# rikuu/Gap2Seq

Measured on AMD Instinct MI355X. Metric: gaps filled/sec (whole node), k=31 synthetic 3 Mbp DBG, higher is better.
Workload: dtype u32

## Files before the change

### gap2seq_amd/csrc/d3_device.h

```cpp
#pragma once
#include <hip/hip_runtime_api.h>
#include <stdint.h>

#include "d2_device.h"
#include "fill_device.h"

#define G2S_D3_BLOCK_VARS 16u
#define G2S_RAND_BLOCK 4096u
#define G2S_RAND_WINDOW 160u
#define G2S_D3_TABLE_BUDGET (8u << 20)

#define G2S_D3_UNHANDLED 0x1u
#define G2S_D3_BUDGET 0x2u
#define G2S_D3_ANOMALY 0x4u

namespace g2s {

struct D3Gap {
  uint64_t arena_off;
  int32_t skip_thr;
  uint16_t lmf;
  uint8_t kind;
  uint8_t pad;
};

struct D3HostItem {
  uint32_t gap, n_segs;
  uint64_t seg_off;
  uint64_t rnd_off;
  uint32_t draws;
  uint32_t pad;
};
struct D3Side {
  D3HostItem* items = nullptr;
  GapOut* outs = nullptr;
  SegRec* segs = nullptr;
  uint32_t* rnd = nullptr;
  uint64_t cap_items = 0, cap_segs = 0, cap_rnd = 0;
  unsigned long long* count = nullptr;
};

struct alignas(16) D3Var {
  uint32_t gap, R, toff, tile0;
  uint32_t base, dmin, dspread, ns;
  uint64_t sub_at;
  uint32_t start_seg, start_t;
  int32_t len0, len1, n_len;
  uint32_t pad;
};
struct alignas(16) D3Trace {
  uint64_t arena_off;
  uint64_t sub_at;
  uint32_t gi;
  uint32_t off, want;
  uint16_t lmf, nsegs;
};
static_assert(sizeof(D3Var) == 64 && sizeof(D3Trace) == 32, "record layouts");

struct D3Summary {
  uint32_t status, unhandled, n_var, anomalies;
  unsigned long long host_items, host_segs, host_rnd;
  uint32_t handoff_waves, tiles;
  uint64_t table_entries, block_entries;
  uint64_t draws_min, draws_spread, draws_total;
  uint64_t xA, sA, xB, sB, xD, sD, segs, fill_bytes;
  uint32_t seg_gaps, filled;
  uint32_t rand_state[31];
  uint32_t trace_waves;
  uint32_t big_gaps;
  uint32_t traced_gaps;
  uint32_t spec_gaps;
  uint32_t handoff_gaps;
};
static_assert(sizeof(D3Summary) <= 512, "the lap stamps live at byte 512 of the summary's slot");

struct RandTables {
  const uint32_t* hi = nullptr;
  const uint32_t* mid = nullptr;
  const uint32_t* lane = nullptr;
};
void rand_tables_host(uint32_t* hi , uint32_t* mid , uint32_t* lane );

struct D3Work {
  uint32_t* ginfo = nullptr;
  uint32_t* dmin = nullptr;
  uint32_t* dspread = nullptr;
  uint32_t* base = nullptr;
  uint32_t* vrank = nullptr;
  uint32_t* var_gap = nullptr;
  uint32_t* var_R = nullptr;
  uint32_t* var_toff = nullptr;
  uint32_t* var_tile = nullptr;
  uint32_t* blk_toff = nullptr;
  uint32_t* blk_in = nullptr;
  uint32_t* dvar = nullptr;
  int32_t* skip = nullptr;
  uint32_t* tile_var = nullptr;
  D3Var* vdesc = nullptr;
  D3Trace* tdesc = nullptr;
  uint32_t* host_slot = nullptr;
  D3HostItem* hitems = nullptr;
  uint16_t* tab = nullptr;
  uint32_t* btab = nullptr;
  D3Summary* sum = nullptr;
  unsigned long long* fill_bytes = nullptr;
  uint32_t* link = nullptr;
  const D2Out* d2out = nullptr;
  const uint32_t* d2runs = nullptr;
  uint64_t* hops = nullptr;
  const char* spec_text = nullptr;
  const uint32_t* spec_res = nullptr;
  uint8_t* tab_bad = nullptr;
};
size_t d3_work_bytes(uint32_t n);
void d3_work_carve(void* p, uint32_t n, D3Work* w);

struct D3Params {
  int32_t k, skip_confident, all_paths, unique_paths;
  uint64_t max_states;
  uint64_t arena_base;
  uint32_t n;
  uint32_t has_skip;
  uint32_t seg_cap;
  uint32_t map_cap;
  uint32_t group_size;
  uint64_t sub_region;
  uint32_t laps;
  uint32_t self_clean;
  uint32_t base0, R0, d_in;
  const unsigned long long* d2_done;
  uint32_t d2_wgs;
  uint32_t restart;
};

hipError_t launch_rand_fill(hipStream_t st, uint32_t* rnd_all, const RandTables& rt, const D3Summary* sum_dev, uint64_t capacity,
                            uint64_t first_value = 0);

hipError_t launch_d3_sharded_classes(hipStream_t st, const D3Params& P, const D3Work& W, const GapOut* outs, const D3Gap* dgaps,
                                     bool summary_is_clean);
hipError_t launch_d3_sharded_tables(hipStream_t st, const D3Params& P, const D3Work& W, const GapOut* outs, const SubRec* sub,
                                    uint32_t* rnd_all, uint64_t rnd_capacity, uint32_t* group_fn );
hipError_t launch_d3_sharded_trace(hipStream_t st, const D3Params& P, const D3Work& W, const GapOut* outs, const SubRec* sub,
                                   const char* lastch_up, const char* lastch_dn, uint32_t* rnd_all, uint64_t rnd_capacity,
                                   void* results, char* arena, const D3Side& side, void* summary_host,
                                   hipEvent_t ev_d2 = nullptr );

hipError_t launch_rand_window(hipStream_t st, uint32_t* rnd_all, const uint32_t* link);

hipError_t launch_d3(hipStream_t st, const D3Params& P, const D3Work& W, const GapDev* gaps, const GapOut* outs,
                     const D3Gap* dgaps, const SubRec* sub, const char* lastch_up, const char* lastch_dn,
                     const RandTables& rt, uint32_t* rnd_all ,
                     uint64_t rnd_capacity, void* results ,
                     char* arena , const D3Side& side ,
                     void* summary_host ,
                     bool summary_is_clean ,
                     uint32_t* clean_words ,
                     hipEvent_t ev_chain = nullptr ,
                     hipEvent_t ev_d2 = nullptr ,
                     hipEvent_t ev_stop = nullptr );

hipError_t test_d3_tables(const uint32_t* segs, uint32_t nsegs, int32_t n_len, int32_t len0, int32_t len1, uint32_t start_seg,
                          const uint32_t* rnd, uint64_t rnd_cap, uint32_t base, uint32_t R, uint32_t dmin, uint32_t dspread,
                          uint16_t* entries, uint8_t* bad, uint32_t* anomalies);

uint64_t d3_chain_launches();

}
```

### gap2seq_amd/csrc/d3_device.hip

```cpp
#include "sync_debug.h"
#include <hip/hip_runtime.h>
#include <hip/hip_ext.h>

#include <algorithm>
#include <atomic>
#include <cstddef>
#include <cstdlib>
#include <cstring>
#include <mutex>
#include <set>
#include <vector>

#include "../../include/g2s.h"
#include "d3_device.h"
#include "envcache.hpp"

namespace {

using g2s::D3Gap;
using g2s::D3Params;
using g2s::D3Summary;
using g2s::D3Work;

__device__ __forceinline__ uint32_t uni(uint32_t x) { return (uint32_t)__builtin_amdgcn_readfirstlane((int)x); }

#define GI_CLASS(x) ((x) & 3u)
#define GI_FILLED 0x4u
#define GI_SKIPPED 0x8u
#define GI_BAD 0x10u
#define GI_MEM 0x20u
#define GI_PHASE_D 0x40u
#define D3_TILE 256u
#define GI_HOST 0x80u

__device__ __forceinline__ void stamp(const D3Work& W, int slot) {
  ((unsigned long long*)((char*)W.sum + 512))[slot] = wall_clock64();
}

__device__ __forceinline__ const SubRec* sub_of(const D3Params& P, const SubRec* sub, uint32_t i) {
  return sub + (uint64_t)(i / P.group_size) * P.sub_region;
}

__device__ __forceinline__ int gap_count(const GapOut& go, const D3Params& P, bool phase_d) {
  if (phase_d && !P.skip_confident && P.all_paths) return go.count_s;
  return go.c_count;
}

__device__ __forceinline__ uint32_t dpp_scan_add(uint32_t x) {
  x += (uint32_t)__builtin_amdgcn_update_dpp(0, (int)x, 0x111, 0xF, 0xF, false);
  x += (uint32_t)__builtin_amdgcn_update_dpp(0, (int)x, 0x112, 0xF, 0xF, false);
  x += (uint32_t)__builtin_amdgcn_update_dpp(0, (int)x, 0x114, 0xF, 0xF, false);
  x += (uint32_t)__builtin_amdgcn_update_dpp(0, (int)x, 0x118, 0xF, 0xF, false);
  x += (uint32_t)__builtin_amdgcn_update_dpp(0, (int)x, 0x142, 0xA, 0xF, false);
  x += (uint32_t)__builtin_amdgcn_update_dpp(0, (int)x, 0x143, 0xC, 0xF, false);
  return x;
}
__device__ __forceinline__ uint32_t sat_add(uint32_t a, uint32_t b) { const uint32_t t = a + b; return t < a ? 0xFFFFFFFFu : t; }
__device__ __forceinline__ uint32_t dpp_scan_sat(uint32_t x) {
  x = sat_add(x, (uint32_t)__builtin_amdgcn_update_dpp(0, (int)x, 0x111, 0xF, 0xF, false));
  x = sat_add(x, (uint32_t)__builtin_amdgcn_update_dpp(0, (int)x, 0x112, 0xF, 0xF, false));
  x = sat_add(x, (uint32_t)__builtin_amdgcn_update_dpp(0, (int)x, 0x114, 0xF, 0xF, false));
  x = sat_add(x, (uint32_t)__builtin_amdgcn_update_dpp(0, (int)x, 0x118, 0xF, 0xF, false));
  x = sat_add(x, (uint32_t)__builtin_amdgcn_update_dpp(0, (int)x, 0x142, 0xA, 0xF, false));
  x = sat_add(x, (uint32_t)__builtin_amdgcn_update_dpp(0, (int)x, 0x143, 0xC, 0xF, false));
  return x;
}
__device__ __forceinline__ uint32_t dpp_sum(uint32_t x) { return (uint32_t)__builtin_amdgcn_readlane((int)dpp_scan_add(x), 63); }
__device__ __forceinline__ unsigned long long wave_add64(unsigned long long v) {
  const unsigned long long lo = dpp_sum((uint32_t)v & 0xFFFFFFu), mid = dpp_sum((uint32_t)(v >> 24) & 0xFFFFFFu), hi = dpp_sum((uint32_t)(v >> 48));
  return lo + (mid << 24) + (hi << 48);
}

__device__ __forceinline__ uint32_t d3_classify_body(const D3Params& P, const D3Work& W, const GapOut* __restrict__ outs,
                                                     const D3Gap* __restrict__ dgaps, uint32_t first, uint32_t stride,
                                                     uint32_t* l_gi, uint32_t* l_dm, uint32_t* l_ds, int32_t* l_sk,
                                                     unsigned long long* red, bool one_wg) {
  const uint32_t n = P.n;
  unsigned long long xA = 0, sA = 0, xB = 0, sB = 0, xD = 0, sD = 0, segs = 0;
  uint32_t unhandled = 0, seg_gaps = 0, big = 0, traced = 0, spec = 0, handoff = 0;
  for (uint32_t i = first; i < n; i += stride) {
    const D3Gap dg = dgaps[i];
    const GapOut& go = outs[i];
    const uint32_t flags = go.flags, n_states = go.n_states, n_right = go.n_right, x_right = go.x_right, x_left = go.x_left;
    const uint32_t x_sub = go.x_sub, n_sub = go.n_sub, nseg_b = go.stat[3], dflags = go.dflags, stop0 = go.stop[0], stop1 = go.stop[1];
    const int c_count = go.c_count, n_len = go.n_len, len0 = go.len[0], len1 = go.len[1], reached_j = go.reached_j, count_s = go.count_s;
    const uint32_t n_xl = go.n_xl;
    const uint64_t sub_off = go.sub_off;
    uint32_t gi = 0, dmin = 0, spread = 0;
    if (dg.kind != 0) gi = GI_BAD;
    else {
      if (flags & (G2S_DEV_OVERFLOW_A | G2S_DEV_OVERFLOW_B)) unhandled++;
      else if ((uint64_t)n_states > P.max_states || (uint64_t)n_right > P.max_states) gi = GI_MEM;
      else {
        xA += x_right; sA += n_right; xB += x_left; sB += n_states; xD += x_sub; sD += n_sub;
        segs += nseg_b;
        seg_gaps++;
        if (flags & G2S_DEV_BIG) big++;
        if (dflags & G2S_DEVA_TRACED) traced++;
        if (dflags & G2S_DEVA_SPEC) spec++;
        const bool phase_d = c_count > 0 && n_len > 0;
        const bool by_host = phase_d && !(dflags & (G2S_DEVA_ANALYSED | G2S_DEVA_D2_PENDING));
        const int cnt = (phase_d && !P.skip_confident && P.all_paths) ? count_s : c_count;
        if (cnt > 0 && (!P.unique_paths || cnt == 1)) gi |= GI_FILLED;
        if (n_len > 0) gi |= ((uint32_t)reached_j & 0xFFu) << 8;
        if (phase_d) {
          gi |= GI_PHASE_D;
          if (by_host) gi |= GI_HOST;
          if (by_host || (!P.skip_confident && (dflags & G2S_DEVA_D2_PENDING))) handoff++;
          int lo_d = 0x7FFFFFFF, hi_d = 0;
#pragma unroll
          for (int q = 0; q < 2; q++) {
            if (q >= n_len) continue;
            const uint32_t sw = q ? stop1 : stop0;
            const int lq = q ? len1 : len0;
            int lo = (int)(sw & 0xFFFFu), hi = (int)(sw >> 16);
            if (lo > hi || hi > (int)dg.lmf) { lo = 0; hi = (int)dg.lmf; }
            lo_d = min(lo_d, 1 + lq - hi);
            hi_d = max(hi_d, 1 + lq - lo);
          }
          lo_d = max(lo_d, 1);
          hi_d = max(hi_d, lo_d);
          dmin = (uint32_t)lo_d;
          spread = (uint32_t)(hi_d - lo_d);
          gi |= spread ? 2u : 1u;
        }
      }
    }
    gi |= (uint32_t)dg.lmf << 16;
    W.ginfo[i] = gi;
    W.dmin[i] = dmin;
    W.dspread[i] = spread;
    W.skip[i] = dg.skip_thr;
    if (l_gi) { l_gi[i] = gi; l_dm[i] = dmin; l_ds[i] = spread; l_sk[i] = dg.skip_thr; }
    uint4 h0;
    const uint64_t ao = P.arena_base + dg.arena_off, sa = (uint64_t)(i / P.group_size) * P.sub_region + sub_off;
    h0.x = (uint32_t)ao; h0.y = (uint32_t)(ao >> 32); h0.z = (uint32_t)sa; h0.w = (uint32_t)(sa >> 32);
    ((uint4*)&W.tdesc[i])[0] = h0;
    (void)n_xl;
  }
  xA = wave_add64(xA); sA = wave_add64(sA); xB = wave_add64(xB); sB = wave_add64(sB); xD = wave_add64(xD); sD = wave_add64(sD);
  segs = wave_add64(segs);
  const unsigned long long cnts = wave_add64(((unsigned long long)unhandled << 32) | seg_gaps);
  big = dpp_sum(big);
  if ((threadIdx.x & 63u) == 0u && big) atomicAdd(&W.sum->big_gaps, big);
  traced = dpp_sum(traced);
  if ((threadIdx.x & 63u) == 0u && traced) atomicAdd(&W.sum->traced_gaps, traced);
  spec = dpp_sum(spec);
  if ((threadIdx.x & 63u) == 0u && spec) atomicAdd(&W.sum->spec_gaps, spec);
  handoff = dpp_sum(handoff);
  if ((threadIdx.x & 63u) == 0u && handoff) atomicAdd(&W.sum->handoff_gaps, handoff);
  const uint32_t wave = threadIdx.x >> 6, nwaves = blockDim.x >> 6;
  if ((threadIdx.x & 63u) == 0u) {
    unsigned long long* r = red + wave * 8u;
    r[0] = xA; r[1] = sA; r[2] = xB; r[3] = sB; r[4] = xD; r[5] = sD; r[6] = segs; r[7] = cnts;
  }
  __syncthreads();
  unsigned long long tot = 0;
  if (threadIdx.x < 8u) for (uint32_t w = 0; w < nwaves; w++) tot += red[w * 8u + threadIdx.x];
  unsigned long long all_cnts = 0;
  for (uint32_t w = 0; w < nwaves; w++) all_cnts += red[w * 8u + 7u];
  D3Summary* S = W.sum;
  if (threadIdx.x < 7u) {
    unsigned long long* dst = (unsigned long long*)&S->xA + threadIdx.x;
    if (one_wg) *dst = tot; else if (tot) atomicAdd(dst, tot);
  } else if (threadIdx.x == 7u) {
    if (one_wg) { S->unhandled = (uint32_t)(tot >> 32); S->seg_gaps = (uint32_t)tot; }
    else {
      if (tot >> 32) atomicAdd(&S->unhandled, (uint32_t)(tot >> 32));
      if (tot & 0xFFFFFFFFull) atomicAdd(&S->seg_gaps, (uint32_t)tot);
    }
  }
  return (uint32_t)(all_cnts >> 32);
}
__global__ __launch_bounds__(256) void g2s_d3_classify(const D3Params P, const D3Work W, const GapOut* __restrict__ outs,
                                                       const D3Gap* __restrict__ dgaps) {
  __shared__ unsigned long long red[4 * 8];
  (void)d3_classify_body(P, W, outs, dgaps, blockIdx.x * blockDim.x + threadIdx.x, gridDim.x * blockDim.x, nullptr, nullptr, nullptr, nullptr, red, false);
}

__device__ __forceinline__ void block_scan3(uint64_t& a, uint64_t& b, uint32_t& c, uint64_t* sh , uint64_t* tot_a, uint64_t* tot_b,
                                            uint32_t* tot_c) {
  const int lane = (int)(threadIdx.x & 63u), wave = (int)(threadIdx.x >> 6);
  uint64_t ia = a, ib = b;
  uint32_t ic = c;
  for (int o = 1; o < 64; o <<= 1) {
    const uint64_t ya = __shfl_up(ia, o), yb = __shfl_up(ib, o);
    const uint32_t yc = __shfl_up(ic, o);
    if (lane >= o) { ia += ya; ib += yb; ic += yc; }
  }
  if (lane == 63) { sh[wave * 3] = ia; sh[wave * 3 + 1] = ib; sh[wave * 3 + 2] = ic; }
  __syncthreads();
  uint64_t wa = lane < 16 ? sh[lane * 3] : 0, wb = lane < 16 ? sh[lane * 3 + 1] : 0, wc = lane < 16 ? sh[lane * 3 + 2] : 0;
  for (int o = 1; o < 16; o <<= 1) {
    const uint64_t ya = __shfl_up(wa, o), yb = __shfl_up(wb, o), yc = __shfl_up(wc, o);
    if (lane >= o) { wa += ya; wb += yb; wc += yc; }
  }
  *tot_a = __shfl(wa, 15); *tot_b = __shfl(wb, 15); *tot_c = (uint32_t)__shfl(wc, 15);
  const uint64_t oa = wave ? __shfl(wa, wave - 1) : 0, ob = wave ? __shfl(wb, wave - 1) : 0, oc = wave ? __shfl(wc, wave - 1) : 0;
  a = oa + ia - a; b = ob + ib - b; c = (uint32_t)oc + ic - c;
}

__device__ __forceinline__ void block_scan3_short(uint32_t& a, uint32_t& b, uint32_t& c, uint32_t* sh , uint32_t* tot_a, uint32_t* tot_b,
                                                  uint32_t* tot_c) {
  const int lane = (int)(threadIdx.x & 63u), wave = (int)(threadIdx.x >> 6);
  const uint32_t ia = dpp_scan_add(a), ib = dpp_scan_add(b), ic = dpp_scan_sat(c);
  if (lane == 63) { sh[wave * 3] = ia; sh[wave * 3 + 1] = ib; sh[wave * 3 + 2] = ic; }
  __syncthreads();
  uint32_t wa = lane < 16 ? sh[lane * 3] : 0u, wb = lane < 16 ? sh[lane * 3 + 1] : 0u, wc = lane < 16 ? sh[lane * 3 + 2] : 0u;
  wa = dpp_scan_add(wa); wb = dpp_scan_add(wb); wc = dpp_scan_sat(wc);
  *tot_a = (uint32_t)__builtin_amdgcn_readlane((int)wa, 15); *tot_b = (uint32_t)__builtin_amdgcn_readlane((int)wb, 15);
  *tot_c = (uint32_t)__builtin_amdgcn_readlane((int)wc, 15);
  const int wp = (int)uni((uint32_t)max(wave - 1, 0));
  const uint32_t oa = wave ? (uint32_t)__builtin_amdgcn_readlane((int)wa, wp) : 0u, ob = wave ? (uint32_t)__builtin_amdgcn_readlane((int)wb, wp) : 0u;
  const uint32_t oc = wave ? (uint32_t)__builtin_amdgcn_readlane((int)wc, wp) : 0u;
  a = oa + ia - a; b = ob + ib - b;
  const uint32_t incl_c = sat_add(oc, ic);
  c = incl_c == 0xFFFFFFFFu ? 0xFFFFFFFFu : incl_c - c;
}

__device__ __forceinline__ void d3_scan_body(const D3Params& P, const D3Work& W, const GapOut* __restrict__ outs, uint32_t* gi_a,
                                             uint32_t* dm_a, uint32_t* ds_a, const int32_t* sk_a, bool dual, uint32_t unhandled,
                                             uint64_t* sh , uint32_t* sh_f , bool short_list ) {
  const uint32_t t = threadIdx.x, n = P.n;
  const uint32_t per = (n + 1023u) / 1024u;
  const uint32_t lo = min(n, t * per), hi = min(n, lo + per);
  if (P.has_skip) {
    auto s_of = [&](uint32_t i) -> bool {
      if (i == 0) return false;
      const int thr = sk_a[i];
      if (thr < 0) return false;
      const uint32_t pg = gi_a[i - 1];
      return (pg & GI_FILLED) && !(pg & (GI_BAD | GI_MEM)) && (int)((pg >> 8) & 0xFFu) > thr;
    };
    bool o0 = false, o1 = true;
    for (uint32_t i = lo; i < hi; i++) { const bool s = s_of(i); o0 = s && !o0; o1 = s && !o1; }
    sh_f[t] = (o0 ? 1u : 0u) | (o1 ? 2u : 0u);
    __syncthreads();
    if (t < 64u) {
      auto apply = [](uint32_t f, bool in) -> bool { return in ? (f & 2u) != 0 : (f & 1u) != 0; };
      uint32_t f = 2u;
      for (uint32_t q = 0; q < 16u; q++) { const uint32_t g = sh_f[t * 16u + q]; f = (apply(g, apply(f, false)) ? 1u : 0u) | (apply(g, apply(f, true)) ? 2u : 0u); }
      uint32_t inc = f;
      for (int o = 1; o < 64; o <<= 1) {
        const uint32_t pv = (uint32_t)__shfl_up((int)inc, o);
        if ((int)t >= o) inc = (apply(inc, apply(pv, false)) ? 1u : 0u) | (apply(inc, apply(pv, true)) ? 2u : 0u);
      }
      uint32_t before = (uint32_t)__shfl_up((int)inc, 1);
      if (t == 0) before = 2u;
      bool cur = apply(before, false);
      for (uint32_t q = 0; q < 16u; q++) { const uint32_t g = sh_f[t * 16u + q]; sh_f[t * 16u + q] = cur ? 1u : 0u; cur = apply(g, cur); }
    }
    __syncthreads();
    bool sk = sh_f[t] != 0;
    for (uint32_t i = lo; i < hi; i++) {
      sk = s_of(i) && !sk;
      if (sk) {
        const uint32_t g = (gi_a[i] & ~3u) | GI_SKIPPED;
        gi_a[i] = g; dm_a[i] = 0; ds_a[i] = 0;
        if (dual) { W.ginfo[i] = g; W.dmin[i] = 0; W.dspread[i] = 0; }
      }
    }
    __threadfence_block();
    __syncthreads();
  }
  auto load8 = [&](uint32_t i0, uint32_t* g8, uint32_t* m8, uint32_t* s8) {
#pragma unroll
    for (int q = 0; q < 8; q++) {
      const uint32_t i = i0 + (uint32_t)q;
      const bool have = i < hi;
      g8[q] = have ? gi_a[i] : GI_SKIPPED;
      m8[q] = have ? dm_a[i] : 0u;
      s8[q] = have ? ds_a[i] : 0u;
    }
  };
  if (t == 0) stamp(W, 20);
  uint64_t sd = 0, ss = 0;
  uint32_t nv = 0;
  for (uint32_t i0 = lo; i0 < hi; i0 += 8u) {
    uint32_t g8[8], m8[8], s8[8];
    load8(i0, g8, m8, s8);
#pragma unroll
    for (int q = 0; q < 8; q++) {
      if (g8[q] & GI_SKIPPED) continue;
      sd += m8[q];
      if (GI_CLASS(g8[q]) == 2u) { nv++; ss += s8[q]; }
    }
  }
  uint64_t tot_d, tot_s;
  uint32_t V;
  if (short_list) {
    uint32_t a = (uint32_t)sd, b = (uint32_t)ss, ta, tb;
    block_scan3_short(a, b, nv, (uint32_t*)sh, &ta, &tb, &V);
    sd = a; ss = b; tot_d = ta; tot_s = tb;
  } else block_scan3(sd, ss, nv, sh, &tot_d, &tot_s, &V);
  if (t == 0) stamp(W, 21);
  const bool too_wide = tot_d + tot_s + P.base0 + P.R0 >= 0xFFFF0000ull || tot_s + P.R0 >= (uint64_t)G2S_D3_TABLE_BUDGET;
  uint64_t my_tab = 0, my_blk = 0;
  uint32_t my_tiles = 0;
  {
    uint64_t d = sd + P.base0, r = ss + P.R0;
    uint32_t v = nv;
    for (uint32_t i0 = lo; i0 < hi; i0 += 8u) {
      uint32_t g8[8], m8[8], s8[8];
      load8(i0, g8, m8, s8);
#pragma unroll
      for (int q = 0; q < 8; q++) {
        const uint32_t i = i0 + (uint32_t)q;
        if (i >= hi) break;
        W.base[i] = (uint32_t)d;
        W.vrank[i] = v;
        if (g8[q] & GI_SKIPPED) continue;
        d += m8[q];
        if (GI_CLASS(g8[q]) == 2u) {
          W.var_gap[v] = i;
          W.var_R[v] = (uint32_t)r;
          my_tab += r + 1u;
          my_tiles += (uint32_t)((r + D3_TILE) / D3_TILE);
          if (v % G2S_D3_BLOCK_VARS == 0u) my_blk += r + 1u;
          v++;
          r += s8[q];
        }
      }
    }
    if (t == 1023u) W.var_R[V] = (uint32_t)tot_s + P.R0;
  }
  if (t == 0) stamp(W, 22);
  uint64_t to = my_tab, bo = my_blk, T, TB;
  uint32_t tl = my_tiles, tiles;
  if (short_list) {
    uint32_t b = (uint32_t)std::min<uint64_t>(bo, 0xFFFFFFFFull), c = (uint32_t)std::min<uint64_t>(to, 0xFFFFFFFFull), tb, tc;
    block_scan3_short(tl, b, c, (uint32_t*)(sh + 48), &tiles, &tb, &tc);
    bo = b; to = c; TB = tb; T = tc == 0xFFFFFFFFu ? ~0ull : tc;
  } else block_scan3(to, bo, tl, sh + 48, &T, &TB, &tiles);
  const bool over = too_wide || T > (uint64_t)G2S_D3_TABLE_BUDGET || TB > (uint64_t)(G2S_D3_TABLE_BUDGET / 4u);
  if (!over) {
    uint64_t d = sd + P.base0, r = ss + P.R0;
    uint32_t v = nv;
    for (uint32_t i0 = lo; i0 < hi; i0 += 8u) {
      uint32_t g8[8], m8[8], s8[8];
      load8(i0, g8, m8, s8);
#pragma unroll
      for (int q = 0; q < 8; q++) {
        if (g8[q] & GI_SKIPPED) continue;
        const uint32_t base_i = (uint32_t)d;
        d += m8[q];
        if (GI_CLASS(g8[q]) != 2u) continue;
        W.var_toff[v] = (uint32_t)to;
        W.var_tile[v] = tl;
        {
          const uint32_t i = i0 + (uint32_t)q;
          uint4 h0, h1;
          h0.x = i; h0.y = (uint32_t)r; h0.z = (uint32_t)to; h0.w = tl;
          h1.x = base_i; h1.y = m8[q]; h1.z = s8[q]; h1.w = 0u;
          ((uint4*)&W.vdesc[v])[0] = h0;
          ((uint4*)&W.vdesc[v])[1] = h1;
        }
        tl += (uint32_t)((r + D3_TILE) / D3_TILE);
        to += r + 1u;
        if (v % G2S_D3_BLOCK_VARS == 0u) { W.blk_toff[v / G2S_D3_BLOCK_VARS] = (uint32_t)bo; bo += r + 1u; }
        v++;
        r += s8[q];
      }
    }
    if (t == 1023u) { W.var_toff[V] = (uint32_t)T; W.var_tile[V] = tiles; W.blk_toff[(V + G2S_D3_BLOCK_VARS - 1u) / G2S_D3_BLOCK_VARS] = (uint32_t)TB; }
    __threadfence_block();
    __syncthreads();
    for (uint32_t v = t; v < V; v += 1024u) {
      const uint4 h0 = ((const uint4*)&W.vdesc[v])[0];
      const uint32_t i = h0.x, r = h0.y, tl0 = h0.w;
      const GapOut& go = outs[i];
      uint4 h2, h3;
      const uint64_t sa = (uint64_t)(i / P.group_size) * P.sub_region + go.sub_off;
      ((uint32_t*)&W.vdesc[v])[7] = go.n_xl;
      h2.x = (uint32_t)sa; h2.y = (uint32_t)(sa >> 32); h2.z = go.start_seg; h2.w = go.start_t;
      h3.x = (uint32_t)go.len[0]; h3.y = (uint32_t)go.len[1]; h3.z = (uint32_t)go.n_len; h3.w = 0u;
      ((uint4*)&W.vdesc[v])[2] = h2;
      ((uint4*)&W.vdesc[v])[3] = h3;
      const uint32_t nt = (r + D3_TILE) / D3_TILE;
      for (uint32_t x = 0; x < nt; x++) W.tile_var[tl0 + x] = v;
    }
  }
  if (t == 0) {
    stamp(W, 23);
    D3Summary* S = W.sum;
    S->status = (unhandled ? G2S_D3_UNHANDLED : 0u) | (over ? G2S_D3_BUDGET : 0u);
    S->n_var = V;
    S->tiles = over ? 0u : tiles;
    S->table_entries = T;
    S->block_entries = TB;
    S->draws_min = tot_d;
    S->draws_spread = tot_s;
  }
}
#define D3_SCAN_LDS_GAPS 12288u
__global__ __launch_bounds__(1024) void g2s_d3_scan(const D3Params P, const D3Work W, const GapOut* __restrict__ outs) {
  extern __shared__ __attribute__((aligned(16))) uint32_t dyn[];
  __shared__ uint64_t sh[96];
  __shared__ uint32_t sh_f[1024];
  if (P.n <= D3_SCAN_LDS_GAPS) {
    uint32_t *l_gi = dyn, *l_dm = dyn + P.n, *l_ds = dyn + 2u * P.n;
    for (uint32_t i = threadIdx.x; i < P.n; i += 1024u) { l_gi[i] = W.ginfo[i]; l_dm[i] = W.dmin[i]; l_ds[i] = W.dspread[i]; }
    const uint32_t unhandled = W.sum->unhandled;
    __syncthreads();
    d3_scan_body(P, W, outs, l_gi, l_dm, l_ds, W.skip, true, unhandled, sh, sh_f, true);
    return;
  }
  d3_scan_body(P, W, outs, W.ginfo, W.dmin, W.dspread, W.skip, false, W.sum->unhandled, sh, sh_f, P.n <= 262144u);
}

__global__ __launch_bounds__(64) void g2s_rand_window(uint32_t* __restrict__ Wd, const uint32_t* __restrict__ link) {
  __shared__ uint32_t w[G2S_RAND_WINDOW + 2];
  const uint32_t lane = threadIdx.x;
  if (lane < 31u) w[lane] = link[lane];
  __syncthreads();
  for (uint32_t i = 31u; i < G2S_RAND_WINDOW; i += 3u) {
    if (lane < 3u) w[i + lane] = w[i + lane - 31u] + w[i + lane - 3u];
    __syncthreads();
  }
  for (uint32_t i = lane; i < G2S_RAND_WINDOW; i += 64u) Wd[i] = w[i];
}
__global__ __launch_bounds__(64) void g2s_rand_fill(uint32_t* __restrict__ Wd, const g2s::RandTables rt, const D3Summary* sum,
                                                    uint64_t capacity, uint64_t first_block) {
  __shared__ uint32_t base[G2S_RAND_WINDOW], s1[96], s2[64];
  if (sum && sum->status) return;
  const uint64_t need = sum ? min(capacity, sum->draws_min + sum->draws_spread + 64ull) : capacity;
  const uint32_t lane = threadIdx.x;
  for (uint32_t i = lane; i < G2S_RAND_WINDOW; i += 64u) base[i] = Wd[i];
  __syncthreads();
  const uint64_t nblocks = (need + G2S_RAND_BLOCK - 1u) / G2S_RAND_BLOCK;
  for (uint64_t B = first_block + blockIdx.x; B < nblocks; B += gridDim.x) {
    const uint32_t* ph = rt.hi + (size_t)((B >> 8) & 127u) * 31u;
    const uint32_t* pm = rt.mid + (size_t)(B & 255u) * 31u;
    const uint32_t* pl = rt.lane + (size_t)lane * 31u;
    for (uint32_t i = lane; i < 91u; i += 64u) {
      uint32_t a = 0;
#pragma unroll
      for (int j = 0; j < 31; j++) a += ph[j] * base[i + (uint32_t)j];
      s1[i] = a;
    }
    __syncthreads();
    if (lane < 61u) {
      uint32_t a = 0;
#pragma unroll
      for (int j = 0; j < 31; j++) a += pm[j] * s1[lane + (uint32_t)j];
      s2[lane] = a;
    }
    __syncthreads();
    uint32_t c[31], r[31];
#pragma unroll
    for (int j = 0; j < 31; j++) c[j] = pl[j];
#pragma unroll
    for (int i = 0; i < 31; i++) {
      uint32_t a = 0;
#pragma unroll
      for (int j = 0; j < 31; j++) a += c[j] * s2[i + j];
      r[i] = a;
    }
    uint32_t* out = Wd + 31u + B * G2S_RAND_BLOCK + (uint64_t)lane * 64u;
    const uint64_t room = capacity > B * G2S_RAND_BLOCK + (uint64_t)lane * 64u ? capacity - (B * G2S_RAND_BLOCK + (uint64_t)lane * 64u) : 0ull;
#pragma unroll
    for (int q = 0; q < 64; q++) {
      const uint32_t v = r[q % 31] + r[(q + 28) % 31];
      r[q % 31] = v;
      if ((uint64_t)q < room) out[q] = v;
    }
    __syncthreads();
  }
}

struct SegW { uint32_t node, depth_len, cnt, ts_tt, par01, par23, flags, pad; };

__device__ __forceinline__ int seg_nparents(uint32_t p01, uint32_t p23) {
  return ((p01 & 0xFFFFu) != 0xFFFFu) + ((p01 >> 16) != 0xFFFFu) + ((p23 & 0xFFFFu) != 0xFFFFu) + ((p23 >> 16) != 0xFFFFu);
}
__device__ __forceinline__ uint32_t seg_parent(uint32_t p01, uint32_t p23, int sel) {
  const uint32_t ps[4] = {p01 & 0xFFFFu, p01 >> 16, p23 & 0xFFFFu, p23 >> 16};
  uint32_t chosen = 0xFFFFu;
  int idx = 0;
#pragma unroll
  for (int q = 0; q < 4; q++)
    if (ps[q] != 0xFFFFu) { if (idx == sel) chosen = ps[q]; idx++; }
  return chosen;
}

__device__ __forceinline__ int pick_parent(uint32_t rv, int nb) { return nb == 2 ? (int)(rv & 1u) : nb == 3 ? (int)(rv % 3u) : (int)(rv & 3u); }

struct SegLite { uint32_t depth_len, par01, par23, flags; };

__device__ __forceinline__ SegLite seg_lite(const SegLite* p, int i) { return p[i]; }
__device__ __forceinline__ SegLite seg_lite(const SegW* p, int i) {
  SegLite l;
  l.depth_len = p[i].depth_len; l.par01 = p[i].par01; l.par23 = p[i].par23; l.flags = p[i].flags;
  return l;
}
template <typename SegT>
__device__ int d3_walk_count(int n_len, int len0, int len1, uint32_t start_seg, uint32_t start_t, int nsegs,
                             const SegT* __restrict__ segs, const uint32_t* lwin ,
                             uint32_t nwin , uint64_t avail ,
                             bool* bad) {
  int draws = 1;
  if (avail < 1 || nwin < 1) { *bad = true; return draws; }
  const int pick = n_len > 1 ? (int)((lwin[0] >> 1) & 1u) : 0;
  int d2 = pick ? len1 : len0;
  const uint32_t sg = (start_seg >> (16 * pick)) & 0xFFFFu;
  int i = sg == 0xFFFFu ? -1 : (int)sg;
  int t = (int)((start_t >> (16 * pick)) & 0xFFFFu);
  if (i < 0 || i >= nsegs) { *bad = true; return draws; }
  SegLite s = seg_lite(segs, i);
  bool ended = false;
  for (int guard = 0; d2 >= 0; guard++) {
    if (guard > 70000) { *bad = true; break; }
    const int run = min(t, d2);
    draws += run; d2 -= run; t -= run;
    if (t == 0 && (s.flags & G2S_SUB_SOURCE)) { ended = true; break; }
    if (d2 > 0) {
      const int nb = seg_nparents(s.par01, s.par23);
      if (nb == 0 || (nb > 1 && !(s.flags & G2S_SEG_ORDERED)) || (uint64_t)draws >= avail || (uint32_t)draws >= nwin) { *bad = true; break; }
      const uint32_t rv = nb > 1 ? lwin[draws] >> 1 : 0u;
      draws++;
      i = (int)seg_parent(s.par01, s.par23, nb == 1 ? 0 : pick_parent(rv, nb));
      if (i >= nsegs) { *bad = true; break; }
      s = seg_lite(segs, i);
      t = (int)(s.depth_len >> 16) - 1;
    }
    d2--;
  }
  if (!ended) *bad = true;
  return draws;
}

template <typename SegT>
__device__ int d3_walk_count_lite(int n_len, int len0, int len1, uint32_t start_seg, int nsegs, const SegT* __restrict__ segs,
                                  const uint32_t* lwin, uint32_t nwin, uint64_t avail, bool* bad) {
  if (avail < 1 || nwin < 1) { *bad = true; return 1; }
  const int pick = n_len > 1 ? (int)((lwin[0] >> 1) & 1u) : 0;
  const int len = pick ? len1 : len0;
  const uint32_t sg = (start_seg >> (16 * pick)) & 0xFFFFu;
  int i = sg == 0xFFFFu ? -1 : (int)sg;
  if (i < 0 || i >= nsegs || len < 0) { *bad = true; return 1; }
  for (int hop = 0; hop <= nsegs; hop++) {
    const SegLite s = seg_lite(segs, i);
    const int d0 = (int)(s.depth_len & 0xFFFFu);
    if (d0 > len) break;
    if (s.flags & G2S_SUB_SOURCE) return 1 + len - d0;
    if (d0 == 0) break;
    const int nb = seg_nparents(s.par01, s.par23);
    const uint32_t at = (uint32_t)(1 + len - d0);
    if (nb == 0 || (nb > 1 && !(s.flags & G2S_SEG_ORDERED)) || (uint64_t)at >= avail || at >= nwin) break;
    const uint32_t rv = nb > 1 ? lwin[at] >> 1 : 0u;
    i = (int)seg_parent(s.par01, s.par23, nb == 1 ? 0 : pick_parent(rv, nb));
    if (i >= nsegs) break;
  }
  *bad = true;
  return 1;
}

__device__ __forceinline__ void wave_lds_sync() {
#ifdef G2S_SYNC_DEBUG
  g2s_sync_jitter(0xD37u);
  g2s_wait_all();
// ... 192 lines not shown
      const uint64_t sub_at = (uint64_t)uni(h2.x) | ((uint64_t)uni(h2.y) << 32);
      const uint64_t at = (uint64_t)base + d;
      bool bad = false;
      const int draws = d3_count_wave((int)uni(h3.z), (int)h3.x, (int)h3.y, h2.z, ns, (const SegW*)(sub + sub_at), rnd + at,
                                      min(win_cap, dmin + dspread + 1u), capacity > at ? capacity - at : 0ull, jmp, dep, &bad);
      if (stw) stamp(W, 6);
      const int dev = draws - (int)dmin;
      if (dev < 0 || dev > (int)dspread) bad = true;
      if ((tid & 63u) == 0u) {
        W.tab[(uint64_t)toff + d] = bad ? (uint16_t)0 : (uint16_t)dev;
        if (W.tab_bad) W.tab_bad[(uint64_t)toff + d] = bad ? 1 : 0;
        bad_any |= bad;
      }
    }
  }
  for (uint32_t tile = blockIdx.x; tile < tiles; tile += gridDim.x) {
    if (by_wave && tile == blockIdx.x && ns_first <= D3_TAB_SEGS) continue;
    const uint32_t v = tile == blockIdx.x ? v_first : W.tile_var[tile];
    const g2s::D3Var vd = W.vdesc[v];
    const uint32_t ns = vd.ns;
    if (by_wave && ns <= D3_TAB_SEGS) continue;
    worked = true;
    const uint32_t d0 = (tile - vd.tile0) * D3_TILE, d = d0 + tid;
    const uint64_t at0 = (uint64_t)vd.base + d0;
    const bool mine = d <= vd.R;
    const uint32_t want = min(win_cap, min(vd.R - d0, D3_TILE - 1u) + vd.dmin + vd.dspread + 1u);
    if (st0 && !by_wave) stamp(W, 5);
    __syncthreads();
    {
      const SegW* gs = (const SegW*)(sub + vd.sub_at);
      const uint32_t in_lds = ns <= D3_TAB_SEGS ? ns : 0u;
#pragma unroll
      for (uint32_t it = 0; it < D3_TAB_SEGS / 256u; it++) {
        const uint32_t q = tid + 256u * it;
        if (q >= in_lds) continue;
        SegLite l;
        l.depth_len = gs[q].depth_len; l.par01 = gs[q].par01; l.par23 = gs[q].par23; l.flags = gs[q].flags;
        lseg[q] = l;
      }
      for (uint32_t x = tid; x < want; x += 256u) lwin[x] = at0 + x < capacity ? rnd[at0 + x] : 0u;
    }
    __syncthreads();
    if (st0 && !by_wave) stamp(W, 6);
    if (mine) {
      bool bad = false;
      const uint64_t at = at0 + tid;
      const uint32_t nw = want > tid ? want - tid : 0u;
      const uint64_t av = capacity > at ? capacity - at : 0ull;
      const int draws = ns > D3_TAB_SEGS
                            ? d3_walk_count(vd.n_len, vd.len0, vd.len1, vd.start_seg, vd.start_t, (int)ns, (const SegW*)(sub + vd.sub_at), lwin + tid, nw, av, &bad)
                            : d3_walk_count_lite(vd.n_len, vd.len0, vd.len1, vd.start_seg, (int)ns, lseg, lwin + tid, nw, av, &bad);
      const int dev = draws - (int)vd.dmin;
      if (dev < 0 || dev > (int)vd.dspread) bad = true;
      W.tab[(uint64_t)vd.toff + d] = bad ? (uint16_t)0 : (uint16_t)dev;
      if (W.tab_bad) W.tab_bad[(uint64_t)vd.toff + d] = bad ? 1 : 0;
      bad_any |= bad;
    }
  }
  if (bad_any) atomicAdd(&W.sum->anomalies, 1u);
  if (st0) stamp(W, 7);
  if (P.laps && (tid & 63u) == 0u) {
    unsigned long long* laps = (unsigned long long*)((char*)W.sum + 512);
    if (worked) atomicMax(&laps[32], wall_clock64());
    if (tid == 0) atomicMax(&laps[33], wall_clock64());
  }
}

__device__ __forceinline__ void d3_blocks_body(const D3Work& W, uint64_t first, uint64_t stride) {
  const D3Summary* S = W.sum;
  const uint32_t V = S->n_var;
  const uint32_t NB = (V + G2S_D3_BLOCK_VARS - 1u) / G2S_D3_BLOCK_VARS;
  const uint64_t TB = S->block_entries;
  for (uint64_t e = first; e < TB; e += stride) {
    uint32_t lo = 0, hi = NB;
    while (hi - lo > 1u) { const uint32_t mid = (lo + hi) >> 1; if ((uint64_t)W.blk_toff[mid] <= e) lo = mid; else hi = mid; }
    const uint32_t b = lo;
    uint32_t d = (uint32_t)(e - W.blk_toff[b]);
    const uint32_t v1 = min(V, (b + 1u) * G2S_D3_BLOCK_VARS);
    for (uint32_t v = b * G2S_D3_BLOCK_VARS; v < v1; v++) d += W.tab[(uint64_t)W.var_toff[v] + d];
    W.btab[e] = d;
  }
}
__global__ __launch_bounds__(256) void g2s_d3_blocks(const D3Work W) {
  if (W.sum->status) return;
  d3_blocks_body(W, (uint64_t)blockIdx.x * blockDim.x + threadIdx.x, (uint64_t)gridDim.x * blockDim.x);
}

__device__ __forceinline__ void d3_chain_body(const D3Work& W, const uint32_t* __restrict__ Wd, uint32_t* total_dev ,
                                              uint32_t base0 = 0u, uint32_t d_in = 0u) {
  D3Summary* S = W.sum;
  const uint32_t V = S->n_var;
  const uint32_t NB = (V + G2S_D3_BLOCK_VARS - 1u) / G2S_D3_BLOCK_VARS;
  __shared__ uint32_t l_toff[2048], l_in[2048];
  const bool in_lds = NB <= 2048u;
  if (in_lds) for (uint32_t b = threadIdx.x; b < NB; b += blockDim.x) l_toff[b] = W.blk_toff[b];
  __syncthreads();
  if (threadIdx.x == 0) {
    uint32_t d = d_in;
    if (in_lds) for (uint32_t b = 0; b < NB; b++) { l_in[b] = d; d = W.btab[(uint64_t)l_toff[b] + d]; }
    else for (uint32_t b = 0; b < NB; b++) { W.blk_in[b] = d; d = W.btab[(uint64_t)W.blk_toff[b] + d]; }
    W.dvar[V] = d;
    *total_dev = d;
  }
  __threadfence_block();
  __syncthreads();
  for (uint32_t b = threadIdx.x; b < NB; b += blockDim.x) {
    uint32_t d = in_lds ? l_in[b] : W.blk_in[b];
    if (in_lds) W.blk_in[b] = d;
    const uint32_t v0 = b * G2S_D3_BLOCK_VARS, v1 = min(V, (b + 1u) * G2S_D3_BLOCK_VARS);
    uint32_t toff[G2S_D3_BLOCK_VARS];
#pragma unroll
    for (uint32_t q = 0; q < G2S_D3_BLOCK_VARS; q++) toff[q] = v0 + q < v1 ? W.var_toff[v0 + q] : 0u;
#pragma unroll
    for (uint32_t q = 0; q < G2S_D3_BLOCK_VARS; q++)
      if (v0 + q < v1) { W.dvar[v0 + q] = d; d += W.tab[(uint64_t)toff[q] + d]; }
  }
  const uint64_t total = (uint64_t)base0 + S->draws_min + *total_dev;
  if (threadIdx.x == 0) S->draws_total = total;
  if (threadIdx.x < 31u) {
    const uint32_t w = Wd[total + threadIdx.x];
    S->rand_state[threadIdx.x] = w;
    if (W.link) W.link[threadIdx.x] = w;
  }
}
__global__ __launch_bounds__(1024) void g2s_d3_chain(const D3Work W, const uint32_t* __restrict__ Wd, uint32_t base0, uint32_t d_in) {
  __shared__ uint32_t total_dev;
  if (W.sum->status) return;
  d3_chain_body(W, Wd, &total_dev, base0, d_in);
}
__global__ __launch_bounds__(256) void g2s_d3_groupfn(const D3Work W, uint32_t R0, uint32_t* __restrict__ fn) {
  const D3Summary* S = W.sum;
  if (S->status) return;
  const uint32_t V = S->n_var;
  const uint32_t NB = (V + G2S_D3_BLOCK_VARS - 1u) / G2S_D3_BLOCK_VARS;
  for (uint32_t d0 = blockIdx.x * blockDim.x + threadIdx.x; d0 <= R0; d0 += gridDim.x * blockDim.x) {
    uint32_t d = d0;
    for (uint32_t b = 0; b < NB; b++) d = W.btab[(uint64_t)W.blk_toff[b] + d];
    fn[d0] = d;
  }
}

#define D3_FRONT_GAPS 3072u
__global__ __launch_bounds__(1024) void g2s_d3_front(const D3Params P, const D3Work W, const GapOut* __restrict__ outs,
                                                     const D3Gap* __restrict__ dgaps) {
  __shared__ uint64_t sh[96];
  __shared__ unsigned long long red[16 * 8];
  __shared__ uint32_t sh_f[1024];
  __shared__ uint32_t l_gi[D3_FRONT_GAPS], l_dm[D3_FRONT_GAPS], l_ds[D3_FRONT_GAPS];
  __shared__ int32_t l_sk[D3_FRONT_GAPS];
  if (threadIdx.x == 0) stamp(W, 0);
  const uint32_t unhandled = d3_classify_body(P, W, outs, dgaps, threadIdx.x, 1024u, l_gi, l_dm, l_ds, l_sk, red, true);
  __syncthreads();
  if (threadIdx.x == 0) stamp(W, 1);
  d3_scan_body(P, W, outs, l_gi, l_dm, l_ds, l_sk, true, unhandled, sh, sh_f, true);
  if (threadIdx.x == 0) stamp(W, 2);
}

template <bool RESTART>
__device__ __forceinline__ bool d3_handoff_body(const D3Params& P, const D3Work& W, const GapOut* __restrict__ outs,
                                                const SubRec* __restrict__ sub, const uint32_t* __restrict__ rnd, uint64_t capacity,
                                                const g2s::D3Side& side, uint32_t i0, const uint32_t* ldvar, const uint16_t* ltab,
                                                const uint32_t* ltoff, unsigned long long* lcur) {
  D3Summary* S = W.sum;
  const int lane = (int)(threadIdx.x & 63u);
  const uint32_t mine = i0 + (uint32_t)lane;
  const bool have = mine < P.n;
  uint32_t gi = 0, my_off = 0, my_want = 0, my_ns = 0;
  if (have) {
    gi = W.ginfo[mine];
    const uint32_t dmin = W.dmin[mine];
    const GapOut& go = outs[mine];
    my_ns = go.n_xl;
    if ((gi & GI_PHASE_D) && !P.skip_confident) {
      const uint32_t dfl = go.dflags;
      if ((dfl & G2S_DEVA_D2_PENDING) && (dfl & G2S_DEVA_D2_FAILED)) gi |= GI_HOST;
    }
    my_want = dmin;
    if constexpr (RESTART) {
      if (GI_CLASS(gi) == 2u) {
        const uint32_t dspread = W.dspread[mine];
        const uint4 h0 = ((const uint4*)&W.tdesc[mine])[0];
        const SegW* gs = (const SegW*)(sub + ((uint64_t)h0.z | ((uint64_t)h0.w << 32)));
        const uint32_t nwin = min(P.map_cap + D3_TILE, dmin + dspread + 1u);
        bool bad = false;
        const int draws = my_ns > D3_TAB_SEGS
                              ? d3_walk_count(go.n_len, go.len[0], go.len[1], go.start_seg, go.start_t, (int)my_ns, gs, rnd, nwin, capacity, &bad)
                              : d3_walk_count_lite(go.n_len, go.len[0], go.len[1], go.start_seg, (int)my_ns, gs, rnd, nwin, capacity, &bad);
        const int dev = draws - (int)dmin;
        if (dev < 0 || dev > (int)dspread) bad = true;
        if (bad) atomicAdd(&S->anomalies, 1u);
        else my_want += (uint32_t)dev;
      }
    } else {
      const uint32_t vr = W.vrank[mine], base = W.base[mine];
      const uint32_t dv = ldvar ? ldvar[vr] : W.dvar[vr];
      my_off = base + dv;
      if (GI_CLASS(gi) == 2u) my_want += ltab ? (uint32_t)ltab[ltoff[vr] + dv] : (uint32_t)W.tab[(uint64_t)W.var_toff[vr] + dv];
    }
    ((uint4*)&W.tdesc[mine])[1] = make_uint4(gi, my_off, my_want, (gi >> 16) | (min(my_ns, 0xFFFFu) << 16));
  }
  const bool host = have && (gi & GI_HOST) != 0u;
  const uint64_t hm = __ballot(host);
  for (uint64_t m = hm; m; m &= m - 1) {
    const int l = __builtin_ctzll(m);
    const uint32_t i = i0 + (uint32_t)l;
    const uint32_t off = (uint32_t)__shfl((int)my_off, l), want = (uint32_t)__shfl((int)my_want, l), ns = (uint32_t)__shfl((int)my_ns, l);
    unsigned long long it = 0, so = 0, ro = 0;
    if (lane == 0) {
      if (lcur) {
        it = atomicAdd(&lcur[0], 1ull); so = atomicAdd(&lcur[1], (unsigned long long)ns); ro = atomicAdd(&lcur[2], ((unsigned long long)want + 8ull) / 8ull);
      } else {
        it = atomicAdd(&S->host_items, 1ull);
        so = atomicAdd(&S->host_segs, (unsigned long long)ns);
        ro = atomicAdd(&S->host_rnd, ((unsigned long long)want + 8ull) / 8ull);
      }
    }
    it = __shfl(it, 0); so = __shfl(so, 0); ro = __shfl(ro, 0);
    if (it >= side.cap_items || so + ns > side.cap_segs || ro + (want + 8ull) / 8ull > side.cap_rnd || (uint64_t)off + want + 1ull > capacity) {
      if (lane == 0) { atomicAdd(&S->anomalies, 1u); W.host_slot[i] = 0xFFFFFFFFu; }
      continue;
    }
    if (lane == 0) {
      g2s::D3HostItem h;
      h.gap = i; h.n_segs = ns; h.seg_off = so; h.rnd_off = ro; h.draws = want; h.pad = 0;
      W.hitems[it] = h;
      W.host_slot[i] = (uint32_t)it;
      uint32_t* hi = (uint32_t*)&side.items[it];
      hi[0] = i; hi[1] = ns; hi[2] = (uint32_t)so; hi[3] = (uint32_t)(so >> 32); hi[4] = (uint32_t)ro; hi[5] = (uint32_t)(ro >> 32); hi[6] = want;
    }
  }
  if (hm != 0ull) __threadfence_system();
  (void)sub; (void)rnd; (void)outs;
  if constexpr (RESTART) {
    const uint32_t nv = (uint32_t)__popcll(__ballot(have && GI_CLASS(gi) == 2u));
    uint32_t mx = have ? my_want : 0u;
    for (int o = 32; o > 0; o >>= 1) mx = max(mx, (uint32_t)__shfl_xor((int)mx, o));
    if (lane == 0) {
      if (nv) atomicAdd(&S->n_var, nv);
      atomicMax((unsigned long long*)&S->draws_total, (unsigned long long)mx);
    }
  }
  return hm != 0ull;
}
__global__ __launch_bounds__(64) void g2s_d3_handoff(const D3Params P, const D3Work W, const GapOut* __restrict__ outs,
                                                     const SubRec* __restrict__ sub, const uint32_t* __restrict__ rnd, uint64_t capacity,
                                                     const g2s::D3Side side) {
  D3Summary* S = W.sum;
  const bool dead = S->status != 0u;
  if (!dead) (void)d3_handoff_body<false>(P, W, outs, sub, rnd, capacity, side, blockIdx.x * 64u, nullptr, nullptr, nullptr, nullptr);
  if ((threadIdx.x & 63u) == 0u) {
    asm volatile("s_waitcnt vmcnt(0)" ::: "memory");
    const unsigned int done = atomicAdd(&S->handoff_waves, 1u) + 1u;
    if (done == gridDim.x) {
      const unsigned long long items = atomicAdd(&S->host_items, 0ull);
      const uint32_t anomalies = atomicAdd(&S->anomalies, 0u);
      __hip_atomic_store(side.count, (items & 0x7FFFFFFFFFFFFFFFull) | ((unsigned long long)((anomalies || dead) ? 1u : 0u) << 63),
                         __ATOMIC_RELEASE, __HIP_MEMORY_SCOPE_SYSTEM);
    }
  }
}
__global__ __launch_bounds__(256) void g2s_d3_restart(const D3Params P, const D3Work W, const GapOut* __restrict__ outs,
                                                      const D3Gap* __restrict__ dgaps, const SubRec* __restrict__ sub,
                                                      const uint32_t* __restrict__ rnd, uint64_t capacity, const g2s::D3Side side) {
  __shared__ unsigned long long red[4 * 8];
  D3Summary* S = W.sum;
  (void)d3_classify_body(P, W, outs, dgaps, blockIdx.x * 256u + threadIdx.x, gridDim.x * 256u, nullptr, nullptr, nullptr, nullptr, red, false);
  (void)d3_handoff_body<true>(P, W, outs, sub, rnd, capacity, side, blockIdx.x * 256u + (threadIdx.x & ~63u), nullptr, nullptr, nullptr, nullptr);
  if ((threadIdx.x & 63u) == 0u) {
    asm volatile("s_waitcnt vmcnt(0)" ::: "memory");
    const unsigned int done = atomicAdd(&S->handoff_waves, 1u) + 1u;
    if (done == gridDim.x * 4u) {
      const unsigned long long items = atomicAdd(&S->host_items, 0ull);
      const uint32_t anomalies = atomicAdd(&S->anomalies, 0u), unhandled = atomicAdd(&S->unhandled, 0u);
      S->status = unhandled ? G2S_D3_UNHANDLED : 0u;
      __hip_atomic_store(side.count, (items & 0x7FFFFFFFFFFFFFFFull) | ((unsigned long long)((anomalies || unhandled) ? 1u : 0u) << 63),
                         __ATOMIC_RELEASE, __HIP_MEMORY_SCOPE_SYSTEM);
    }
  }
}
#define D3_BACK_TAB 24576u
#define D3_CHAIN_GAPS 768u
#define D3_CHAIN_ROOM 4096u
__global__ __launch_bounds__(1024) void g2s_d3_back(const D3Params P, const D3Work W, const GapOut* __restrict__ outs,
                                                    const SubRec* __restrict__ sub, const uint32_t* __restrict__ Wd, uint64_t capacity,
                                                    const g2s::D3Side side) {
  __shared__ uint32_t total_dev;
  __shared__ unsigned long long lcur[3];
  if (threadIdx.x < 3u) lcur[threadIdx.x] = 0ull;
  __shared__ uint16_t ltab[D3_BACK_TAB];
  __shared__ uint32_t ltoff[1025], ldvar[1025];
  D3Summary* S = W.sum;
  if (threadIdx.x == 0) stamp(W, 8);
  const uint32_t status = S->status, V = S->n_var;
  const uint64_t T = S->table_entries;
  if (status) {
    if (threadIdx.x == 0) __hip_atomic_store(side.count, 1ull << 63, __ATOMIC_RELEASE, __HIP_MEMORY_SCOPE_SYSTEM);
    return;
  }
  const bool in_lds = T <= (uint64_t)D3_BACK_TAB && V <= 1024u;
  if (in_lds) {
    for (uint32_t e = threadIdx.x; e < (uint32_t)T; e += 1024u) ltab[e] = W.tab[e];
    if (threadIdx.x <= V) ltoff[threadIdx.x] = W.var_toff[threadIdx.x];
    __syncthreads();
    if (threadIdx.x == 0) {
      stamp(W, 9);
      uint32_t d = 0;
      for (uint32_t v = 0; v < V; v++) { ldvar[v] = d; d += ltab[ltoff[v] + d]; }
      ldvar[V] = d;
// ... 713 lines not shown
         ((size_t)n + 64) * (sizeof(D3Var) + sizeof(D3Trace) + sizeof(D3HostItem)) + ((size_t)n + G2S_D3_TABLE_BUDGET / 256u + 64) * 4;
}

void d3_work_carve(void* p, uint32_t n, D3Work* w) {
  char* c = (char*)p;
  const size_t per = (((size_t)n + 64) * 4 + 63) & ~(size_t)63;
  w->sum = (D3Summary*)c; c += 1024;
  w->fill_bytes = (unsigned long long*)c; c += 64 * 128;
  w->ginfo = (uint32_t*)c; c += per;
  w->dmin = (uint32_t*)c; c += per;
  w->dspread = (uint32_t*)c; c += per;
  w->base = (uint32_t*)c; c += per;
  w->vrank = (uint32_t*)c; c += per;
  w->var_gap = (uint32_t*)c; c += per;
  w->var_R = (uint32_t*)c; c += per;
  w->var_toff = (uint32_t*)c; c += per;
  w->var_tile = (uint32_t*)c; c += per;
  w->blk_toff = (uint32_t*)c; c += per;
  w->blk_in = (uint32_t*)c; c += per;
  w->dvar = (uint32_t*)c; c += per;
  w->skip = (int32_t*)c; c += per;
  w->host_slot = (uint32_t*)c; c += per;
  w->vdesc = (D3Var*)c; c += ((size_t)n + 64) * sizeof(D3Var);
  w->tdesc = (D3Trace*)c; c += ((size_t)n + 64) * sizeof(D3Trace);
  w->hitems = (D3HostItem*)c; c += ((size_t)n + 64) * sizeof(D3HostItem);
  w->tile_var = (uint32_t*)c; c += ((size_t)n + G2S_D3_TABLE_BUDGET / 256u + 64) * 4;
  w->btab = (uint32_t*)c; c += (size_t)(G2S_D3_TABLE_BUDGET / 4u) * 4;
  w->tab = (uint16_t*)c;
}

hipError_t launch_rand_fill(hipStream_t st, uint32_t* rnd_all, const RandTables& rt, const D3Summary* sum_dev, uint64_t capacity,
                            uint64_t first_value) {
  const uint64_t first_block = first_value / G2S_RAND_BLOCK;
  const uint64_t all = (capacity + G2S_RAND_BLOCK - 1) / G2S_RAND_BLOCK;
  const uint32_t rblocks = (uint32_t)std::min<uint64_t>(all > first_block ? all - first_block : 1, 4096);
  hipLaunchKernelGGL(g2s_rand_fill, dim3(std::max(1u, rblocks)), dim3(64), 0, st, rnd_all, rt, sum_dev, capacity, first_block);
  return hipGetLastError();
}

static void launch_scan(hipStream_t st, const D3Params& P, const D3Work& W, const GapOut* outs) {
  static std::mutex mu;
  static std::set<int> done;
  int dev = 0;
  (void)hipGetDevice(&dev);
  {
    std::lock_guard<std::mutex> lk(mu);
    if (done.insert(dev).second)
      (void)hipFuncSetAttribute((const void*)g2s_d3_scan, hipFuncAttributeMaxDynamicSharedMemorySize, (int)(12u * D3_SCAN_LDS_GAPS));
  }
  const size_t lds = P.n <= D3_SCAN_LDS_GAPS ? 12u * (size_t)P.n : 0u;
  hipLaunchKernelGGL(g2s_d3_scan, dim3(1), dim3(1024), lds, st, P, W, outs);
}

static hipError_t launch_tables(hipStream_t st, const D3Params& P, const D3Work& W, const SubRec* sub, uint32_t* rnd_all, uint64_t rnd_capacity) {
  const size_t win = ((size_t)P.map_cap + D3_TILE) * 4;
  const bool waves = P.n <= D3_FRONT_GAPS;
  const hipError_t e = hipFuncSetAttribute(waves ? (const void*)g2s_d3_tables_waves : (const void*)g2s_d3_tables, hipFuncAttributeMaxDynamicSharedMemorySize, (int)win);
  if (e != hipSuccess) return e;
  if (waves) hipLaunchKernelGGL(g2s_d3_tables_waves, dim3(D3_WAVE_GRID), dim3(256), win, st, P, W, sub, rnd_all + 31, rnd_capacity);
  else hipLaunchKernelGGL(g2s_d3_tables, dim3(std::min(8192u, std::max(128u, P.n / 2u))), dim3(256), win, st, P, W, sub, rnd_all + 31, rnd_capacity);
  return hipGetLastError();
}

hipError_t test_d3_tables(const uint32_t* segs, uint32_t nsegs, int32_t n_len, int32_t len0, int32_t len1, uint32_t start_seg,
                          const uint32_t* rnd, uint64_t rnd_cap, uint32_t base, uint32_t R, uint32_t dmin, uint32_t dspread,
                          uint16_t* entries, uint8_t* bad, uint32_t* anomalies) {
  const uint32_t tiles = (R + D3_TILE) / D3_TILE;
  const size_t n_tile_var = 8192u + tiles, n_rnd = 31u + (size_t)rnd_cap + 64u;
  std::vector<SegW> hs(std::max(nsegs, 1u));
  for (uint32_t q = 0; q < nsegs; q++) {
    SegW w = {};
    w.depth_len = segs[4u * q]; w.par01 = segs[4u * q + 1u]; w.par23 = segs[4u * q + 2u]; w.flags = segs[4u * q + 3u];
    hs[q] = w;
  }
  std::vector<uint32_t> hr(n_rnd, 0u);
  for (uint64_t x = 0; x < rnd_cap; x++) hr[31u + x] = rnd[x];
  D3Var vd = {};
  vd.gap = 0; vd.R = R; vd.toff = 0; vd.tile0 = 0; vd.base = base; vd.dmin = dmin; vd.dspread = dspread; vd.ns = nsegs;
  auto start_t = [&](int pick) -> uint32_t {
    const uint32_t sg = (start_seg >> (16 * pick)) & 0xFFFFu;
    const int t = sg < nsegs ? (pick ? len1 : len0) - (int)(segs[4u * sg] & 0xFFFFu) : 0;
    return t >= 0 && t <= 0xFFFF ? (uint32_t)t : 0u;
  };
  vd.sub_at = 0; vd.start_seg = start_seg; vd.start_t = start_t(0) | (start_t(1) << 16); vd.len0 = len0; vd.len1 = len1; vd.n_len = n_len;
  D3Summary sum = {};
  sum.n_var = 1; sum.tiles = tiles; sum.table_entries = (uint64_t)R + 1u;
  void *d_sum = nullptr, *d_vd = nullptr, *d_tv = nullptr, *d_seg = nullptr, *d_rnd = nullptr, *d_tab = nullptr, *d_bad = nullptr;
  auto release = [&]() { for (void* p : {d_sum, d_vd, d_tv, d_seg, d_rnd, d_tab, d_bad}) if (p) (void)hipFree(p); };
  hipError_t e = hipSuccess;
  auto ok = [&](hipError_t x) { if (e == hipSuccess) e = x; return e == hipSuccess; };
  if (ok(hipMalloc(&d_sum, 1024)) && ok(hipMalloc(&d_vd, 4 * sizeof(D3Var))) && ok(hipMalloc(&d_tv, n_tile_var * 4)) &&
      ok(hipMalloc(&d_seg, hs.size() * sizeof(SegW))) && ok(hipMalloc(&d_rnd, n_rnd * 4)) && ok(hipMalloc(&d_tab, ((size_t)R + 1u) * 2)) &&
      ok(hipMalloc(&d_bad, (size_t)R + 1u)) && ok(hipMemset(d_sum, 0, 1024)) && ok(hipMemset(d_vd, 0, 4 * sizeof(D3Var))) &&
      ok(hipMemset(d_tv, 0, n_tile_var * 4)) && ok(hipMemset(d_tab, 0xFF, ((size_t)R + 1u) * 2)) && ok(hipMemset(d_bad, 0xFF, (size_t)R + 1u)) &&
      ok(hipMemcpy(d_sum, &sum, sizeof sum, hipMemcpyHostToDevice)) && ok(hipMemcpy(d_vd, &vd, sizeof vd, hipMemcpyHostToDevice)) &&
      ok(hipMemcpy(d_seg, hs.data(), hs.size() * sizeof(SegW), hipMemcpyHostToDevice)) &&
      ok(hipMemcpy(d_rnd, hr.data(), n_rnd * 4, hipMemcpyHostToDevice))) {
    D3Params P;
    memset(&P, 0, sizeof P);
    P.n = 1; P.group_size = 1;
    P.map_cap = ((uint32_t)std::max(std::max(len0, len1), 0) + 2u + 3u) & ~3u;
    D3Work W;
    W.sum = (D3Summary*)d_sum; W.vdesc = (D3Var*)d_vd; W.tile_var = (uint32_t*)d_tv; W.tab = (uint16_t*)d_tab; W.tab_bad = (uint8_t*)d_bad;
    if (ok(launch_tables(nullptr, P, W, (const SubRec*)d_seg, (uint32_t*)d_rnd, rnd_cap)) && ok(hipDeviceSynchronize()) &&
        ok(hipMemcpy(entries, d_tab, ((size_t)R + 1u) * 2, hipMemcpyDeviceToHost)) && ok(hipMemcpy(bad, d_bad, (size_t)R + 1u, hipMemcpyDeviceToHost)) &&
        ok(hipMemcpy(&sum, d_sum, sizeof sum, hipMemcpyDeviceToHost)))
      *anomalies = sum.anomalies;
  }
  release();
  return e;
}

hipError_t launch_rand_window(hipStream_t st, uint32_t* rnd_all, const uint32_t* link) {
  hipLaunchKernelGGL(g2s_rand_window, dim3(1), dim3(64), 0, st, rnd_all, link);
  return hipGetLastError();
}

hipError_t launch_d3_sharded_classes(hipStream_t st, const D3Params& P, const D3Work& W, const GapOut* outs, const D3Gap* dgaps,
                                     bool summary_is_clean) {
  if (P.n == 0) return hipSuccess;
  hipError_t e = summary_is_clean ? hipSuccess : hipMemsetAsync(W.sum, 0, 1024 + 64 * 128, st);
  if (e != hipSuccess) return e;
  hipLaunchKernelGGL(g2s_d3_classify, dim3((P.n + 255u) / 256u), dim3(256), 0, st, P, W, outs, dgaps);
  launch_scan(st, P, W, outs);
  return hipGetLastError();
}
hipError_t launch_d3_sharded_tables(hipStream_t st, const D3Params& P, const D3Work& W, const GapOut* outs, const SubRec* sub,
                                    uint32_t* rnd_all, uint64_t rnd_capacity, uint32_t* group_fn) {
  if (P.n == 0) return hipSuccess;
  launch_scan(st, P, W, outs);
  const hipError_t e = launch_tables(st, P, W, sub, rnd_all, rnd_capacity);
  if (e != hipSuccess) return e;
  hipLaunchKernelGGL(g2s_d3_blocks, dim3(256), dim3(256), 0, st, W);
  hipLaunchKernelGGL(g2s_d3_groupfn, dim3(std::min(256u, (P.R0 + 256u) / 256u)), dim3(256), 0, st, W, P.R0, group_fn);
  return hipGetLastError();
}
hipError_t launch_d3_sharded_trace(hipStream_t st, const D3Params& P, const D3Work& W, const GapOut* outs, const SubRec* sub,
                                   const char* lastch_up, const char* lastch_dn, uint32_t* rnd_all, uint64_t rnd_capacity,
                                   void* results, char* arena, const D3Side& side, void* summary_host, hipEvent_t ev_d2) {
  if (P.n == 0) return hipSuccess;
  hipLaunchKernelGGL(g2s_d3_chain, dim3(1), dim3(1024), 0, st, W, rnd_all, P.base0, P.d_in);
  if (ev_d2) { const hipError_t e2 = hipStreamWaitEvent(st, ev_d2, 0); if (e2 != hipSuccess) return e2; }
  hipLaunchKernelGGL(g2s_d3_handoff, dim3((P.n + 63u) / 64u), dim3(64), 0, st, P, W, outs, sub, rnd_all + 31, rnd_capacity, side);
  const size_t lds = (size_t)P.seg_cap * (sizeof(SegRec) + 16) + (size_t)P.map_cap * 8 + 16;
  hipError_t e = hipFuncSetAttribute((const void*)g2s_d3_trace<1>, hipFuncAttributeMaxDynamicSharedMemorySize, (int)lds);
  if (e != hipSuccess) return e;
  hipLaunchKernelGGL(g2s_d3_trace<1>, dim3(P.n), dim3(64), lds, st, P, W, const_cast<GapOut*>(outs), sub, lastch_up, lastch_dn, rnd_all + 31, rnd_capacity,
                     (g2s_result*)results, arena, (uint32_t*)summary_host, side, (uint32_t*)nullptr, 0u);
  return hipGetLastError();
}

static std::atomic<uint64_t> chain_launches{0};
uint64_t d3_chain_launches() { return chain_launches.load(std::memory_order_relaxed); }

hipError_t launch_d3(hipStream_t st, const D3Params& P, const D3Work& W, const GapDev* gaps, const GapOut* outs,
                     const D3Gap* dgaps, const SubRec* sub, const char* lastch_up, const char* lastch_dn,
                     const RandTables& rt, uint32_t* rnd_all, uint64_t rnd_capacity, void* results, char* arena,
                     const D3Side& side, void* summary_host, bool summary_is_clean, uint32_t* clean_words, hipEvent_t ev_chain,
                     hipEvent_t ev_d2, hipEvent_t ev_stop) {
  if (P.n == 0) return hipSuccess;
  (void)gaps;
  (void)rt;
  static_assert(sizeof(D3Summary) <= 1024, "summary slot");
  hipError_t e = summary_is_clean ? hipSuccess : hipMemsetAsync(W.sum, 0, 1024 + 64 * 128, st);
  if (e != hipSuccess) return e;
  const bool short_list = P.n <= D3_FRONT_GAPS;
  if (P.restart) {
    if (ev_d2) { e = hipStreamWaitEvent(st, ev_d2, 0); if (e != hipSuccess) return e; }
    hipLaunchKernelGGL(g2s_d3_restart, dim3((P.n + 255u) / 256u), dim3(256), 0, st, P, W, outs, dgaps, sub, rnd_all + 31, rnd_capacity, side);
  } else if (short_list) hipLaunchKernelGGL(g2s_d3_front, dim3(1), dim3(1024), 0, st, P, W, outs, dgaps);
  else {
    hipLaunchKernelGGL(g2s_d3_classify, dim3((P.n + 255u) / 256u), dim3(256), 0, st, P, W, outs, dgaps);
    launch_scan(st, P, W, outs);
  }
  if (!P.restart) { e = launch_tables(st, P, W, sub, rnd_all, rnd_capacity); if (e != hipSuccess) return e; }
  if (ev_d2 && short_list && !P.restart) { e = hipStreamWaitEvent(st, ev_d2, 0); if (e != hipSuccess) return e; }
  const char* waves_s = GENV("G2S_TRACE_WAVES");
  const int waves_env = waves_s ? atoi(waves_s) : 0;
  const bool four = waves_env ? waves_env == 4 : P.n <= 768u;
  const size_t lds = (size_t)P.seg_cap * (sizeof(SegRec) + 16) + (size_t)P.map_cap * 8 + 16;
  bool chain_in_trace = false;
  uint32_t chain_room = 0;
  static_assert(D3_CHAIN_GAPS <= 768u, "g2s_d3_trace<4, true> is the four-wave kernel");
  if (!P.restart && four && P.n <= D3_CHAIN_GAPS && ev_chain == nullptr && P.group_size >= P.n && !P.base0 && !P.R0 && !P.d_in) {
    const char* back_s = GENV("G2S_D3_BACK");
    chain_in_trace = !(back_s && atoi(back_s) != 0);
    const char* room_s = GENV("G2S_TEST_CHAIN_ROOM");
    chain_room = (uint32_t)std::min<size_t>(lds / 2u, 0x7FFFFFFFu);
    if (room_s) chain_room = std::min(chain_room, (uint32_t)std::max(atoi(room_s), 0));
  }
  if (P.restart) (void)ev_chain;
  else if (chain_in_trace) (void)ev_chain;
  else if (short_list) {
    hipLaunchKernelGGL(g2s_d3_back, dim3(1), dim3(1024), 0, st, P, W, outs, sub, rnd_all, rnd_capacity, side);
    if (ev_chain) { e = hipEventRecord(ev_chain, st); if (e != hipSuccess) return e; }
  } else {
    hipLaunchKernelGGL(g2s_d3_blocks, dim3(256), dim3(256), 0, st, W);
    hipLaunchKernelGGL(g2s_d3_chain, dim3(1), dim3(1024), 0, st, W, rnd_all, 0u, 0u);
    if (ev_chain) { e = hipEventRecord(ev_chain, st); if (e != hipSuccess) return e; }
    if (ev_d2) { e = hipStreamWaitEvent(st, ev_d2, 0); if (e != hipSuccess) return e; }
    hipLaunchKernelGGL(g2s_d3_handoff, dim3((P.n + 63u) / 64u), dim3(64), 0, st, P, W, outs, sub, rnd_all + 31, rnd_capacity, side);
  }
  e = hipFuncSetAttribute(chain_in_trace ? (const void*)g2s_d3_trace<4, true> : four ? (const void*)g2s_d3_trace<4> : (const void*)g2s_d3_trace<1>,
                          hipFuncAttributeMaxDynamicSharedMemorySize, (int)lds);
  if (e != hipSuccess) return e;
  if (chain_in_trace) {
    chain_launches.fetch_add(1, std::memory_order_relaxed);
    if (ev_stop != nullptr)
      hipExtLaunchKernelGGL((g2s_d3_trace<4, true>), dim3(P.n), dim3(256), (uint32_t)lds, st, nullptr, ev_stop, 0u, P, W, const_cast<GapOut*>(outs), sub, lastch_up, lastch_dn,
                            rnd_all + 31, rnd_capacity, (g2s_result*)results, arena, (uint32_t*)summary_host, side, clean_words, chain_room);
    else
      hipLaunchKernelGGL((g2s_d3_trace<4, true>), dim3(P.n), dim3(256), lds, st, P, W, const_cast<GapOut*>(outs), sub, lastch_up, lastch_dn, rnd_all + 31, rnd_capacity,
                         (g2s_result*)results, arena, (uint32_t*)summary_host, side, clean_words, chain_room);
    return hipGetLastError();
  }
  if (ev_stop != nullptr) {
    if (four)
      hipExtLaunchKernelGGL(g2s_d3_trace<4>, dim3(P.n), dim3(256), (uint32_t)lds, st, nullptr, ev_stop, 0u, P, W, const_cast<GapOut*>(outs), sub, lastch_up, lastch_dn,
                            rnd_all + 31, rnd_capacity, (g2s_result*)results, arena, (uint32_t*)summary_host, side, clean_words, 0u);
    else
      hipExtLaunchKernelGGL(g2s_d3_trace<1>, dim3(P.n), dim3(64), (uint32_t)lds, st, nullptr, ev_stop, 0u, P, W, const_cast<GapOut*>(outs), sub, lastch_up, lastch_dn,
                            rnd_all + 31, rnd_capacity, (g2s_result*)results, arena, (uint32_t*)summary_host, side, clean_words, 0u);
    return hipGetLastError();
  }
  if (four)
    hipLaunchKernelGGL(g2s_d3_trace<4>, dim3(P.n), dim3(256), lds, st, P, W, const_cast<GapOut*>(outs), sub, lastch_up, lastch_dn, rnd_all + 31, rnd_capacity,
                       (g2s_result*)results, arena, (uint32_t*)summary_host, side, clean_words, 0u);
  else
    hipLaunchKernelGGL(g2s_d3_trace<1>, dim3(P.n), dim3(64), lds, st, P, W, const_cast<GapOut*>(outs), sub, lastch_up, lastch_dn, rnd_all + 31, rnd_capacity,
                       (g2s_result*)results, arena, (uint32_t*)summary_host, side, clean_words, 0u);
  return hipGetLastError();
}

}
```

### gap2seq_amd/csrc/g2s_api.hip

```cpp
#include <hip/hip_runtime.h>
#include <cstdarg>
#include <sys/prctl.h>
#include <pthread.h>
#include <sched.h>
#include <time.h>

#include <algorithm>
#include <atomic>
#include <chrono>
#include <cstdio>
#include <cstdlib>
#include <condition_variable>
#include <cstring>
#include <functional>
#include <mutex>
#include <string>
#include <thread>
#include <vector>

#include "../../include/g2s.h"
#include "../../include/g2s_test.h"
#include "envcache.hpp"
#include "d2_device.h"
#include "d3_device.h"
// ... 4872 lines not shown
  return G2S_OK;
}

extern "C" int64_t g2s_graph_validate(const g2s_graph* gr, char* msg, size_t msg_cap) {
  if (!gr || !gr->g) return -1;
  const Graph& g = *gr->g;
  std::string text;
  int64_t bad = 0;
  auto note = [&](const char* what, uint64_t i) {
    if (bad++ < 8) text += std::string(what) + " at k-mer " + std::to_string(i) + "; ";
  };
  auto only = [&](uint32_t v, uint32_t want) {
    int cnt = 0;
    bool hit = false;
    for (int nt = 0; nt < 4; nt++) {
      const uint32_t w = g.succ_of(v, nt);
      if (w == kInvalidNode) continue;
      cnt++;
      hit = hit || w == want;
    }
    return cnt == 1 && hit;
  };
  uint64_t starts = 0;
  for (uint64_t i = 0; i < g.n; i++) {
    const bool start = (g.ustart[i >> 6] >> (i & 63)) & 1;
    starts += start;
    if (i == 0) { if (!start) note("first k-mer is not a unitig start", i); continue; }
    if (start) continue;
    const uint32_t a = (uint32_t)(2 * (i - 1)), b = (uint32_t)(2 * i);
    if (!only(a, b)) note("internal edge is not the only successor (even orientation)", i);
    if (!only(b ^ 1u, a ^ 1u)) note("internal edge is not the only successor (odd orientation)", i);
  }
  if (starts != g.n_unitigs) note("bitmap population differs from the unitig count", starts);
  if (!g.set_lo.empty()) {
    if (g.set_lo.front() != 0 || g.set_lo.back() != g.n) note("set ranges do not cover the k-mers", g.n);
    for (size_t s = 0; s + 1 < g.set_lo.size(); s++) {
      if (g.set_lo[s] > g.set_lo[s + 1]) { note("set ranges not ascending", g.set_lo[s]); continue; }
      for (uint64_t i = g.set_lo[s]; i < g.set_lo[s + 1]; i++)
        for (uint32_t v = (uint32_t)(2 * i); v <= (uint32_t)(2 * i + 1); v++)
          for (int nt = 0; nt < 4; nt++) {
            const uint32_t w = g.succ_of(v, nt);
            if (w != kInvalidNode && ((w >> 1) < g.set_lo[s] || (w >> 1) >= g.set_lo[s + 1])) note("successor outside its set", i);
          }
    }
  }
  for (uint64_t v = 0; v < 2 * g.n; v++)
    for (int nt = 0; nt < 4; nt++) {
      const uint32_t w = g.succ_of((uint32_t)v, nt);
      if (w == kInvalidNode) continue;
      if (w >= 2 * g.n) { note("successor out of range", v >> 1); continue; }
      if (g.lastnt[w] != nt) note("last base of a successor differs from its slot", v >> 1);
    }
  if (msg && msg_cap) {
    const size_t c = std::min(text.size(), msg_cap - 1);
    memcpy(msg, text.data(), c);
    msg[c] = 0;
  }
  return bad;
}

extern "C" int g2s_test_worker_pool(int32_t threads, int32_t rounds, int32_t n) {
  if (threads < 1 || rounds < 0 || n < 0) return fail(G2S_ERR_ARG, "g2s_test_worker_pool: bad argument");
  WorkerPool pool(threads - 1);
  std::vector<std::atomic<int>> hits((size_t)n);
  for (int r = 0; r < rounds; r++) {
    for (auto& h : hits) h.store(0);
    std::atomic<long long> sum(0);
    const int nn = (r % 7 == 0) ? std::min(n, 3) : n;
    pool.run((size_t)nn, [&](size_t i) { hits[i].fetch_add(1); sum.fetch_add((long long)i + 1); });
    if (sum.load() != (long long)nn * (nn + 1) / 2) return fail(G2S_ERR_STATE, "worker pool: wrong task sum");
    for (int i = 0; i < nn; i++)
      if (hits[(size_t)i].load() != 1) return fail(G2S_ERR_STATE, "worker pool: task not run exactly once");
  }
  return G2S_OK;
}

extern "C" int g2s_test_group_queue(int32_t nworkers, uint64_t n, uint64_t group_size, int32_t* owner) {
  return g2s_test_group_queue_slow(nworkers, n, group_size, -1, 0, owner);
}
extern "C" int g2s_test_group_queue_slow(int32_t nworkers, uint64_t n, uint64_t group_size, int32_t slow_worker,
                                         uint32_t slow_us, int32_t* owner) {
  if (nworkers < 1 || !owner) return fail(G2S_ERR_ARG, "g2s_test_group_queue: bad argument");
  for (uint64_t i = 0; i < n; i++) owner[i] = -1;
  GroupQueue queue((size_t)n, (size_t)group_size);
  std::atomic<int> clash(0);
  auto worker = [&](int t) {
    size_t gi = 0, off = 0, cnt = 0;
    while (queue.pull(&gi, &off, &cnt)) {
      for (size_t i = off; i < off + cnt; i++) { if (owner[i] != -1) clash.fetch_add(1); owner[i] = t; }
      std::this_thread::sleep_for(std::chrono::microseconds(20 + (t == slow_worker ? slow_us : 0u)));
    }
  };
  std::vector<std::thread> th;
  for (int t = 1; t < nworkers; t++) th.emplace_back(worker, t);
  worker(0);
  for (auto& x : th) x.join();
  if (clash.load()) return fail(G2S_ERR_STATE, "group queue: a gap was handed out twice");
  for (uint64_t i = 0; i < n; i++) if (owner[i] < 0) return fail(G2S_ERR_STATE, "group queue: a gap was never handed out");
  return G2S_OK;
}

extern "C" int g2s_test_device_rand(int device, uint32_t seed, uint64_t skip, uint32_t n, int32_t* out) {
  if (!out) return fail(G2S_ERR_ARG, "g2s_test_device_rand: bad argument");
  int ndev = 0;
  if (hipGetDeviceCount(&ndev) != hipSuccess || device < 0 || device >= ndev) return fail(G2S_ERR_NO_DEVICE, "no such device");
  HIP_TRY(hipSetDevice(device));
  GlibcRandStream st;
  st.seed(seed);
  for (uint64_t left = skip; left;) {
    const size_t c = (size_t)std::min<uint64_t>(left, 1u << 20);
    st.ensure(c);
    st.consume(c);
    left -= c;
  }
  std::vector<uint32_t> tables((128 + 256 + 64) * 31);
  rand_tables_host(tables.data(), tables.data() + 128 * 31, tables.data() + (128 + 256) * 31);
  const uint64_t cap = ((uint64_t)n + 2 * G2S_RAND_BLOCK) & ~(uint64_t)(G2S_RAND_BLOCK - 1);
  uint32_t *d_tab = nullptr, *d_rnd = nullptr;
  D3Summary* d_sum = nullptr;
  HIP_TRY(hipMalloc((void**)&d_tab, tables.size() * 4));
  HIP_TRY(hipMalloc((void**)&d_rnd, (31 + cap + 64) * 4));
  HIP_TRY(hipMalloc((void**)&d_sum, sizeof(D3Summary)));
  D3Summary sum;
  memset(&sum, 0, sizeof sum);
  sum.draws_min = n;
  HIP_TRY(hipMemcpy(d_tab, tables.data(), tables.size() * 4, hipMemcpyHostToDevice));
  HIP_TRY(hipMemcpy(d_sum, &sum, sizeof sum, hipMemcpyHostToDevice));
  HIP_TRY(hipMemcpy(d_rnd, st.window(G2S_RAND_WINDOW), G2S_RAND_WINDOW * 4, hipMemcpyHostToDevice));
  RandTables rt;
  rt.hi = d_tab; rt.mid = d_tab + 128 * 31; rt.lane = d_tab + (128 + 256) * 31;
  HIP_TRY(launch_rand_fill(nullptr, d_rnd, rt, d_sum, cap));
  HIP_TRY(hipDeviceSynchronize());
  std::vector<uint32_t> h(n);
  HIP_TRY(hipMemcpy(h.data(), d_rnd + 31, (size_t)n * 4, hipMemcpyDeviceToHost));
  for (uint32_t i = 0; i < n; i++) out[i] = (int32_t)(h[i] >> 1);
  (void)hipFree(d_tab); (void)hipFree(d_rnd); (void)hipFree(d_sum);
  return G2S_OK;
}

extern "C" int g2s_test_d3_tables(int device, const uint32_t* segs, uint32_t n_segs, int32_t n_len, int32_t len0, int32_t len1,
                                  uint32_t start_seg, const uint32_t* rnd, uint64_t rnd_cap, uint32_t base, uint32_t R, uint32_t dmin,
                                  uint32_t dspread, uint16_t* entries, uint8_t* bad, uint32_t* anomalies) {
  if ((!segs && n_segs) || (!rnd && rnd_cap) || !entries || !bad || !anomalies || n_segs > 0xFFFFu || n_len < 1 || n_len > 2 ||
      (uint64_t)R + 1u > (uint64_t)G2S_D3_TABLE_BUDGET)
    return fail(G2S_ERR_ARG, "g2s_test_d3_tables: bad argument");
  int ndev = 0;
  if (hipGetDeviceCount(&ndev) != hipSuccess || device < 0 || device >= ndev) return fail(G2S_ERR_NO_DEVICE, "no such device");
  HIP_TRY(hipSetDevice(device));
  HIP_TRY(test_d3_tables(segs, n_segs, n_len, len0, len1, start_seg, rnd, rnd_cap, base, R, dmin, dspread, entries, bad, anomalies));
  return G2S_OK;
}

extern "C" uint64_t g2s_test_d3_chain_launches(void) { return d3_chain_launches(); }

extern "C" int g2s_test_rand_skip(uint32_t seed, uint64_t skip, uint32_t n, int32_t* out) {
  if (!out) return fail(G2S_ERR_ARG, "g2s_test_rand_skip: bad argument");
  GlibcRandStream st;
  st.seed(seed);
  st.skip(skip);
  st.ensure(n);
  for (uint32_t i = 0; i < n; i++) out[i] = st.value(i);
  return G2S_OK;
}
extern "C" int g2s_test_rand_stream(uint32_t seed, uint32_t skip, uint32_t n, int32_t* out) {
  if (!out) return fail(G2S_ERR_ARG, "g2s_test_rand_stream: bad argument");
  GlibcRandStream st;
  st.seed(seed);
  st.ensure(skip / 2 + 1);
  st.consume(skip / 2);
  st.ensure(skip - skip / 2 + n);
  st.consume(skip - skip / 2);
  for (uint32_t i = 0; i < n; i++) out[i] = st.value(i);
  return G2S_OK;
}
```

### gap2seq_amd/lib.py

```python
import ctypes as C
import os

G2S_OK = 0
G2S_ERR_IO = -2
G2S_ERR_NO_DEVICE = -3
G2S_ERR_STATE = -6
G2S_INVALID_NODE = 0xFFFFFFFF
G2S_MAX_PATHS = 2147483647 // 2 - 1
G2S_MAX_IN_FLIGHT = 3
G2S_GROUP_PER_SESSION = (1 << 64) - 1
G2S_GAP_SKIPPED = 0x1
G2S_GAP_Q7 = 0x2
G2S_GAP_MEM_EXCEEDED = 0x4
G2S_GAP_BACKTRACE_FAIL = 0x8
G2S_GAP_BAD_FLANK = 0x10
G2S_GAP_PHASE_D = 0x20


class G2SError(RuntimeError):
    def __init__(self, code, msg):
        super().__init__("g2s error %d: %s" % (code, msg))
        self.code = code


# ... 61 lines not shown
                ("ms_join", C.c_double), ("ms_text", C.c_double)]


class g2s_read_pool(C.Structure):
    _fields_ = [("n_reads", C.c_uint64), ("bases", C.POINTER(C.c_char)), ("base_off", C.POINTER(C.c_uint64)),
                ("names", C.POINTER(C.c_char)), ("name_off", C.POINTER(C.c_uint64)), ("gap_begin", C.POINTER(C.c_uint64)),
                ("gap_read", C.POINTER(C.c_uint32)), ("n_unmapped", C.c_uint64), ("unmapped_read", C.POINTER(C.c_uint32))]


_VP = C.c_void_p
TEXT_FN = C.CFUNCTYPE(None, C.POINTER(C.c_char), C.c_size_t, C.c_void_p)
_SIGS = {
    "g2s_abi_version": (C.c_int, []),
    "g2s_fill_begin": (C.c_int, [_VP, C.POINTER(g2s_gap), C.c_size_t, C.POINTER(g2s_result), C.c_void_p, C.c_size_t]),
    "g2s_fill_end": (C.c_int, [_VP]),
    "g2s_fill_in_flight": (C.c_int, [_VP]),
    "g2s_share_begin": (C.c_int, [_VP, C.POINTER(g2s_gap), C.c_size_t, C.POINTER(g2s_result), C.c_void_p, C.c_size_t,
                                  C.POINTER(C.c_uint64)]),
    "g2s_share_tables": (C.c_int, [_VP, C.c_uint64, C.c_uint64, C.POINTER(C.POINTER(C.c_uint32))]),
    "g2s_share_trace": (C.c_int, [_VP, C.c_uint32]),
    "g2s_share_end": (C.c_int, [_VP, C.c_uint64]),
    "g2s_backtrace_text": (C.c_size_t, [C.POINTER(g2s_gap), C.POINTER(g2s_result), C.c_int, C.c_char_p, C.c_size_t]),
    "g2s_last_error": (C.c_char_p, []),
    "g2s_graph_build_files": (C.c_int, [C.c_char_p, C.c_int, C.c_int, C.c_int, C.POINTER(_VP)]),
    "g2s_graph_build_seqs": (C.c_int, [C.POINTER(C.c_char_p), C.POINTER(C.c_uint64), C.c_int, C.c_int, C.c_int,
                                       C.c_int, C.POINTER(_VP)]),
    "g2s_graph_build_sets": (C.c_int, [C.POINTER(C.c_char_p), C.POINTER(C.c_uint64), C.POINTER(C.c_uint32), C.c_int,
                                       C.c_uint32, C.c_int, C.c_int, C.c_int, C.POINTER(_VP)]),
    "g2s_graph_build_pool": (C.c_int, [C.POINTER(C.c_char_p), C.POINTER(C.c_uint64), C.c_uint64, C.POINTER(C.c_uint64),
                                       C.POINTER(C.c_uint32), C.POINTER(C.c_uint32), C.c_uint64, C.POINTER(C.c_uint8),
                                       C.c_uint32, C.c_int, C.c_int, C.c_int, C.POINTER(_VP)]),
    "g2s_graph_build_pool_reach": (C.c_int, [C.POINTER(C.c_char_p), C.POINTER(C.c_uint64), C.c_uint64, C.POINTER(C.c_uint64),
                                             C.POINTER(C.c_uint32), C.POINTER(C.c_uint32), C.c_uint64, C.POINTER(C.c_uint8),
                                             C.c_uint32, C.c_int, C.c_int, C.c_int, C.POINTER(g2s_gap), C.POINTER(C.c_int32),
                                             C.POINTER(_VP)]),
    "g2s_graph_build_seqs_reach": (C.c_int, [C.POINTER(C.c_char_p), C.POINTER(C.c_uint64), C.c_int, C.c_int, C.c_int, C.c_int,
                                             C.POINTER(g2s_gap), C.POINTER(C.c_int32), C.c_uint64, C.c_int, C.POINTER(_VP)]),
    "g2s_graph_build_files_reach": (C.c_int, [C.c_char_p, C.c_int, C.c_int, C.c_int, C.POINTER(g2s_gap), C.POINTER(C.c_int32),
                                              C.c_uint64, C.c_int, C.POINTER(_VP)]),
    "g2s_scaffolds_reach": (C.c_int, [C.c_char_p, C.c_int, C.c_int, C.c_int, C.POINTER(_VP)]),
    "g2s_reach_records_count": (C.c_uint64, [_VP]),
    "g2s_reach_records_gaps": (C.POINTER(g2s_gap), [_VP]),
    "g2s_reach_records_radii": (C.POINTER(C.c_int32), [_VP]),
    "g2s_reach_records_free": (None, [_VP]),
    "g2s_graph_bounded": (C.c_int, [_VP]),
    "g2s_test_last_graph_reach": (C.c_int, [C.POINTER(C.c_uint64)] * 5 + [C.POINTER(C.c_uint32)] * 3 + [C.POINTER(C.c_int),
                                                                                                                  C.POINTER(C.c_double)]),
    "g2s_test_last_pool_reach": (C.c_int, [C.POINTER(C.c_uint64), C.POINTER(C.c_uint64), C.POINTER(C.c_int), C.POINTER(C.c_uint64),
                                           C.POINTER(C.c_uint32), C.POINTER(C.c_int)]),
    "g2s_test_last_pool_build": (C.c_int, [C.POINTER(C.c_uint64), C.POINTER(C.c_uint64), C.POINTER(C.c_uint64),
                                           C.POINTER(C.c_int)]),
    "g2s_test_last_solid_count": (C.c_int, [C.POINTER(C.c_uint64), C.POINTER(C.c_uint32), C.POINTER(C.c_uint32),
                                            C.POINTER(C.c_uint64), C.POINTER(C.c_uint64), C.POINTER(C.c_int)]),
    "g2s_test_plan_passes": (C.c_int, [C.POINTER(C.c_uint64), C.c_uint32, C.c_uint64, C.POINTER(C.c_uint32), C.c_uint32,
                                       C.POINTER(C.c_uint32), C.POINTER(C.c_uint32)]),
    "g2s_test_seg_back_record": (C.c_int, [_VP, C.c_int, C.c_uint32, C.POINTER(C.c_uint32)]),
    "g2s_graph_num_sets": (C.c_uint32, [_VP]),
    "g2s_graph_set_nodes": (C.c_int, [_VP, C.c_uint32, C.POINTER(C.c_uint64), C.POINTER(C.c_uint64)]),
    "g2s_graph_set_node": (C.c_uint32, [_VP, C.c_uint32, C.c_char_p]),
    "g2s_graph_save": (C.c_int, [_VP, C.c_char_p]),
    "g2s_graph_load": (C.c_int, [C.c_char_p, C.POINTER(_VP)]),
    "g2s_graph_free": (None, [_VP]),
    "g2s_graph_k": (C.c_int, [_VP]),
    "g2s_graph_solid": (C.c_int, [_VP]),
    "g2s_graph_num_kmers": (C.c_uint64, [_VP]),
    "g2s_graph_num_unitigs": (C.c_uint64, [_VP]),
    "g2s_graph_node": (C.c_uint32, [_VP, C.c_char_p]),
    "g2s_graph_successors": (C.c_int, [_VP, C.c_uint32, C.POINTER(C.c_uint32)]),
    "g2s_graph_predecessors": (C.c_int, [_VP, C.c_uint32, C.POINTER(C.c_uint32)]),
    "g2s_graph_node_string": (C.c_int, [_VP, C.c_uint32, C.c_char_p]),
    "g2s_graph_upload": (C.c_int, [_VP, C.c_int]),
    "g2s_graph_device_bytes": (C.c_uint64, [_VP, C.c_int]),
    "g2s_session_create": (C.c_int, [_VP, C.c_int, C.POINTER(g2s_params), C.POINTER(_VP)]),
    "g2s_session_destroy": (None, [_VP]),
    "g2s_session_srand": (C.c_int, [_VP, C.c_uint32]),
    "g2s_session_skip_draws": (C.c_int, [_VP, C.c_uint64]),
    "g2s_session_graph": (_VP, [_VP]),
    "g2s_session_get_params": (C.c_int, [_VP, C.POINTER(g2s_params)]),
    "g2s_batch_prepare": (C.c_int, [_VP, C.POINTER(g2s_gap), C.c_size_t, C.POINTER(_VP)]),
    "g2s_batch_run": (C.c_int, [_VP, C.POINTER(g2s_result), C.c_char_p, C.c_size_t]),
    "g2s_batch_arena_bytes": (C.c_size_t, [_VP]),
    "g2s_batch_timing": (C.c_int, [_VP, C.POINTER(g2s_timing)]),
    "g2s_batch_free": (None, [_VP]),
    "g2s_session_last_timing": (C.c_int, [_VP, C.POINTER(g2s_timing)]),
    "g2s_fill_batch": (C.c_int, [_VP, C.POINTER(g2s_gap), C.c_size_t, C.POINTER(g2s_result), C.c_char_p,
                                 C.c_size_t]),
    "g2s_team_fill": (C.c_int, [C.POINTER(_VP), C.c_int, C.POINTER(g2s_gap), C.c_size_t, C.c_size_t,
                                C.POINTER(g2s_result), C.c_char_p, C.c_size_t, C.POINTER(g2s_timing)]),
    "g2s_team_arena_bytes": (C.c_size_t, [_VP, C.POINTER(g2s_gap), C.c_size_t]),
    "g2s_fill_sets": (C.c_int, [_VP, C.POINTER(g2s_gap), C.POINTER(C.c_uint32), C.c_size_t, C.POINTER(g2s_result),
                                C.c_char_p, C.c_size_t]),
    "g2s_session_set_team": (C.c_int, [_VP, C.POINTER(_VP), C.c_int, C.c_size_t]),
    "g2s_execute_scaffolds_stream": (C.c_int, [_VP, C.POINTER(g2s_run_opts), C.c_char_p, C.c_char_p, C.c_char_p, C.c_size_t,
                                             TEXT_FN, TEXT_FN, _VP, C.POINTER(C.c_int32), C.POINTER(C.c_int32)]),
    "g2s_execute_scaffolds": (C.c_int, [_VP, C.POINTER(g2s_run_opts), C.c_char_p, C.c_char_p, C.c_char_p,
                                        C.POINTER(_VP), C.POINTER(_VP), C.POINTER(C.c_int32),
                                        C.POINTER(C.c_int32)]),
    "g2s_execute_single": (C.c_int, [_VP, C.POINTER(g2s_run_opts), C.c_char_p, C.c_char_p, C.c_char_p, C.c_char_p,
                                     C.c_int32, C.POINTER(_VP), C.POINTER(_VP)]),
    "g2s_free": (None, [_VP]),
    "g2s_host_alloc": (_VP, [C.c_size_t]),
    "g2s_host_free": (None, [_VP]),
    "g2s_cut_scaffolds": (C.c_int, [C.c_char_p, C.c_int, C.c_int, C.c_int, C.c_int, C.c_char_p, C.c_char_p, C.c_char_p,
                                    C.c_char_p, C.POINTER(_VP), C.POINTER(_VP), C.POINTER(_VP), C.POINTER(_VP)]),
    "g2s_merge_scaffolds": (C.c_int, [C.c_char_p, C.c_char_p, C.c_char_p, C.c_char_p, C.c_char_p, C.POINTER(_VP),
                                      C.POINTER(_VP)]),
    "g2s_filter_reads": (C.c_int, [C.c_char_p, C.POINTER(g2s_filter_opts), C.POINTER(_VP), C.POINTER(_VP),
                                   C.POINTER(_VP), C.POINTER(C.c_int64), C.POINTER(C.c_int64)]),
    "g2s_filter_reads_mem": (C.c_int, [C.c_char_p, C.c_size_t, C.POINTER(g2s_filter_opts), C.POINTER(_VP),
                                       C.POINTER(_VP), C.POINTER(_VP), C.POINTER(C.c_int64), C.POINTER(C.c_int64)]),
    "g2s_filter_reads_gaps": (C.c_int, [C.c_char_p, C.POINTER(g2s_filter_opts), C.POINTER(g2s_filter_gap), C.c_size_t,
                                        C.c_int, C.POINTER(_VP), C.POINTER(_VP), C.POINTER(_VP), C.POINTER(C.c_int64),
                                        C.POINTER(C.c_int64), C.POINTER(_VP), C.POINTER(C.c_int64),
                                        C.POINTER(g2s_filter_stats)]),
    "g2s_filter_reads_gaps_mem": (C.c_int, [C.c_char_p, C.c_size_t, C.POINTER(g2s_filter_opts), C.POINTER(g2s_filter_gap),
                                            C.c_size_t, C.c_int, C.POINTER(_VP), C.POINTER(_VP), C.POINTER(_VP),
                                            C.POINTER(C.c_int64), C.POINTER(C.c_int64), C.POINTER(_VP),
                                            C.POINTER(C.c_int64), C.POINTER(g2s_filter_stats)]),
    "g2s_filter_reads_gaps_pool": (C.c_int, [C.c_char_p, C.POINTER(g2s_filter_opts), C.POINTER(g2s_filter_gap), C.c_size_t,
                                             C.c_int, C.c_int, C.c_int, C.POINTER(C.POINTER(g2s_read_pool)),
                                             C.POINTER(C.c_int64), C.POINTER(g2s_filter_stats)]),
    "g2s_filter_reads_gaps_pool_mem": (C.c_int, [C.c_char_p, C.c_size_t, C.POINTER(g2s_filter_opts), C.POINTER(g2s_filter_gap),
                                                 C.c_size_t, C.c_int, C.c_int, C.c_int, C.POINTER(C.POINTER(g2s_read_pool)),
                                                 C.POINTER(C.c_int64), C.POINTER(g2s_filter_stats)]),
    "g2s_read_pool_free": (None, [C.POINTER(g2s_read_pool)]),
    "g2s_filter_reads_gaps_dpool": (C.c_int, [C.c_char_p, C.POINTER(g2s_filter_opts), C.POINTER(g2s_filter_gap), C.c_size_t,
                                              C.c_int, C.c_int, C.POINTER(_VP), C.POINTER(C.c_int64),
                                              C.POINTER(g2s_filter_stats)]),
    "g2s_filter_reads_gaps_dpool_mem": (C.c_int, [C.c_char_p, C.c_size_t, C.POINTER(g2s_filter_opts), C.POINTER(g2s_filter_gap),
                                                  C.c_size_t, C.c_int, C.c_int, C.POINTER(_VP), C.POINTER(C.c_int64),
                                                  C.POINTER(g2s_filter_stats)]),
    "g2s_device_pool_view": (C.POINTER(g2s_read_pool), [_VP]),
    "g2s_device_pool_device": (C.c_int, [_VP]),
    "g2s_device_pool_bytes": (C.c_uint64, [_VP]),
    "g2s_device_pool_read": (C.c_int, [_VP, C.c_uint64, C.c_char_p]),
    "g2s_device_pool_free": (None, [_VP]),
    "g2s_graph_build_dpool_reach": (C.c_int, [C.POINTER(_VP), C.c_uint32, C.POINTER(C.c_uint64), C.POINTER(C.c_uint32),
                                              C.POINTER(C.c_uint32), C.c_uint64, C.POINTER(C.c_uint8), C.c_uint32, C.c_int,
                                              C.c_int, C.c_int, C.POINTER(g2s_gap), C.POINTER(C.c_int32), C.POINTER(_VP)]),
    "g2s_test_last_dpool": (C.c_int, [C.POINTER(C.c_int), C.POINTER(C.c_uint64), C.POINTER(C.c_uint64),
                                      C.POINTER(C.c_uint64)]),
    "g2s_filter_last_error": (C.c_char_p, []),
    "g2s_device_count": (C.c_int, []),
    "g2s_synth_genome": (C.c_int, [C.c_uint64, C.c_uint32, C.c_uint64, C.POINTER(_VP)]),
    "g2s_synth_gaps": (C.c_int, [C.c_char_p, C.c_int, C.c_int, C.c_int, C.c_int, C.c_int, C.c_uint64,
                                 C.POINTER(_VP)]),
    "g2s_test_rand_skip": (C.c_int, [C.c_uint32, C.c_uint64, C.c_uint32, C.POINTER(C.c_int32)]),
    "g2s_test_rand_stream": (C.c_int, [C.c_uint32, C.c_uint32, C.c_uint32, C.POINTER(C.c_int32)]),
    "g2s_test_device_rand": (C.c_int, [C.c_int, C.c_uint32, C.c_uint64, C.c_uint32, C.POINTER(C.c_int32)]),
    "g2s_test_d3_tables": (C.c_int, [C.c_int, C.POINTER(C.c_uint32), C.c_uint32, C.c_int32, C.c_int32, C.c_int32, C.c_uint32,
                                     C.POINTER(C.c_uint32), C.c_uint64, C.c_uint32, C.c_uint32, C.c_uint32, C.c_uint32,
                                     C.POINTER(C.c_uint16), C.POINTER(C.c_uint8), C.POINTER(C.c_uint32)]),
    "g2s_test_d3_chain_launches": (C.c_uint64, []),
    "g2s_test_post_closure": (C.c_int, [_VP, C.POINTER(g2s_params), C.POINTER(g2s_gap), C.c_uint32,
                                        C.POINTER(C.c_uint32), C.c_uint32, C.POINTER(C.c_uint64), C.c_int32, C.c_int32,
                                        C.POINTER(C.c_int32), C.c_int32, C.c_int32, C.c_uint32, C.c_uint64,
                                        C.POINTER(g2s_result), C.c_char_p]),
    "g2s_test_graph_tables": (C.c_int, [_VP, C.POINTER(C.c_uint32), C.POINTER(C.c_uint64)]),
    "g2s_test_post_segments": (C.c_int, [_VP, C.POINTER(g2s_params), C.POINTER(g2s_gap), C.c_uint32,
                                         C.POINTER(C.c_uint32), C.c_int32, C.c_int32, C.POINTER(C.c_int32), C.c_int32,
                                         C.c_int32, C.c_uint32, C.c_uint64, C.POINTER(g2s_result), C.c_char_p,
                                         C.POINTER(C.c_int32)]),
    "g2s_test_seg_expand": (C.c_int, [_VP, C.POINTER(g2s_params), C.POINTER(g2s_gap), C.c_uint32, C.POINTER(C.c_uint32),
                                      C.c_int32, C.POINTER(C.c_int32), C.c_int32, C.c_uint32, C.POINTER(C.c_uint32),
                                      C.c_uint32, C.POINTER(C.c_uint64)]),
    "g2s_test_worker_pool": (C.c_int, [C.c_int32, C.c_int32, C.c_int32]),
    "g2s_test_group_queue": (C.c_int, [C.c_int32, C.c_uint64, C.c_uint64, C.POINTER(C.c_int32)]),
    "g2s_test_group_queue_slow": (C.c_int, [C.c_int32, C.c_uint64, C.c_uint64, C.c_int32, C.c_uint32, C.POINTER(C.c_int32)]),
    "g2s_test_filter_join": (C.c_int, [C.c_int, C.c_int32, C.c_uint64, C.POINTER(C.c_int32), C.POINTER(C.c_int32),
                                       C.POINTER(C.c_int64), C.POINTER(C.c_uint32), C.POINTER(C.c_uint64),
                                       C.POINTER(C.c_uint64), C.c_int64, C.c_uint64, C.c_uint64, C.POINTER(C.c_int64),
                                       C.c_uint64, C.POINTER(C.c_uint64), C.c_uint64, C.POINTER(C.c_uint64),
                                       C.POINTER(C.c_uint64), C.c_uint64, C.POINTER(C.c_uint64)]),
    "g2s_test_reads_text": (C.c_int, [C.c_char_p, C.c_size_t, C.c_int, C.c_size_t, C.POINTER(C.c_uint8), C.c_size_t,
                                      C.POINTER(C.c_size_t)]),
    "g2s_test_last_reads_load": (C.c_int, [C.POINTER(C.c_uint64), C.POINTER(C.c_uint64), C.POINTER(C.c_uint64),
                                           C.POINTER(C.c_uint64), C.POINTER(C.c_uint64), C.POINTER(C.c_int),
                                           C.POINTER(C.c_int), C.c_uint64, C.POINTER(C.c_uint64)]),
    "g2s_test_last_reads_bam": (C.c_int, [C.POINTER(C.c_uint64), C.POINTER(C.c_uint64), C.POINTER(C.c_uint64),
                                          C.POINTER(C.c_int), C.POINTER(C.c_int), C.POINTER(C.c_int)]),
    "g2s_test_last_reads_bam_stream": (C.c_int, [C.POINTER(C.c_uint64), C.POINTER(C.c_uint64), C.POINTER(C.c_uint64)]),
    "g2s_test_bgzf_inflate": (C.c_int, [C.c_char_p, C.c_size_t, C.c_int, C.POINTER(C.c_uint8), C.c_size_t,
                                        C.POINTER(C.c_size_t), C.POINTER(C.c_int64)]),
    "g2s_test_last_filter_inflate": (C.c_int, [C.POINTER(C.c_int), C.POINTER(C.c_uint64), C.POINTER(C.c_uint64),
                                               C.POINTER(C.c_uint64), C.POINTER(C.c_double), C.POINTER(C.c_double)]),
    "g2s_test_bam_rows": (C.c_int, [C.c_char_p, C.c_size_t, C.c_int, C.c_size_t, C.c_uint64, C.POINTER(C.c_int32),
                                    C.POINTER(C.c_int32), C.POINTER(C.c_int64), C.POINTER(C.c_uint32), C.POINTER(C.c_uint64),
                                    C.POINTER(C.c_uint64), C.POINTER(C.c_uint64), C.POINTER(C.c_int32), C.POINTER(C.c_int64)]),
    "g2s_test_bam_rows_kept": (C.c_int, [C.c_char_p, C.c_size_t, C.c_int, C.c_size_t, C.c_uint64, C.POINTER(C.c_int32),
                                         C.POINTER(C.c_int32), C.POINTER(C.c_int64), C.POINTER(C.c_uint32), C.POINTER(C.c_uint64),
                                         C.POINTER(C.c_uint64), C.POINTER(C.c_uint64), C.POINTER(C.c_int32), C.POINTER(C.c_int64)]),
    "g2s_test_name_hash": (C.c_int, [C.c_char_p, C.c_size_t, C.c_int, C.POINTER(C.c_uint64), C.POINTER(C.c_uint64)]),
    "g2s_test_last_filter_rows": (C.c_int, [C.POINTER(C.c_int), C.POINTER(C.c_uint64), C.POINTER(C.c_uint64),
                                            C.POINTER(C.c_uint64), C.POINTER(C.c_int)]),
    "g2s_filter_set_one_pass": (C.c_int, [C.c_int]),
    "g2s_reads_set_device_gzip": (C.c_int, [C.c_int]),
    "g2s_test_gzip_inflate": (C.c_int, [C.c_char_p, C.c_size_t, C.c_int, C.c_uint32, C.c_uint32, C.POINTER(C.c_uint8),
                                        C.c_size_t, C.POINTER(C.c_size_t), C.POINTER(C.c_int)]),
    "g2s_test_last_reads_gzip": (C.c_int, [C.POINTER(C.c_uint64), C.POINTER(C.c_uint64), C.POINTER(C.c_uint64),
                                           C.POINTER(C.c_uint64), C.POINTER(C.c_uint64), C.POINTER(C.c_uint64),
                                           C.POINTER(C.c_int), C.POINTER(C.c_uint64)]),
    "g2s_test_last_filter_text": (C.c_int, [C.POINTER(C.c_int), C.POINTER(C.c_int), C.POINTER(C.c_uint64), C.POINTER(C.c_uint64),
                                            C.POINTER(C.c_uint64)]),
    "g2s_test_bam_text": (C.c_int, [C.c_char_p, C.c_size_t, C.c_int, C.POINTER(C.c_uint32), C.c_uint64, C.c_int, C.c_int,
                                    C.POINTER(C.c_uint8), C.c_uint64, C.POINTER(C.c_uint64), C.POINTER(C.c_uint8), C.c_uint64,
                                    C.POINTER(C.c_uint64), C.POINTER(C.c_uint64), C.POINTER(C.c_uint64), C.c_uint64,
                                    C.POINTER(C.c_uint64)]),
    "g2s_test_bam_text_store": (C.c_int, [C.c_char_p, C.c_size_t, C.c_int, C.c_size_t, C.POINTER(C.c_uint32), C.c_uint64, C.c_int,
                                          C.c_int, C.POINTER(C.c_uint8), C.c_uint64, C.POINTER(C.c_uint64), C.POINTER(C.c_uint8),
                                          C.c_uint64, C.POINTER(C.c_uint64), C.POINTER(C.c_uint64), C.POINTER(C.c_uint64),
                                          C.c_uint64, C.POINTER(C.c_uint64)]),
    "g2s_test_filter_store_plan": (C.c_int, [C.c_char_p, C.c_size_t] + [C.POINTER(C.c_uint64)] * 6),
    "g2s_test_bam_store": (C.c_int, [C.c_char_p, C.c_size_t, C.c_int, C.c_size_t, C.POINTER(C.c_uint8), C.c_uint64,
                                     C.POINTER(C.c_uint64), C.POINTER(C.c_uint64), C.c_uint64, C.POINTER(C.c_uint64)]),
    "g2s_test_last_filter_store": (C.c_int, [C.POINTER(C.c_int)] + [C.POINTER(C.c_uint64)] * 5 + [C.POINTER(C.c_int)]),
    "g2s_graph_validate": (C.c_int64, [C.c_void_p, C.c_char_p, C.c_size_t]),
    "g2s_test_post_gap": (C.c_int, [_VP, C.POINTER(g2s_params), C.POINTER(g2s_gap), C.c_int32,
                                    C.POINTER(C.c_uint32), C.POINTER(C.c_int32), C.POINTER(C.c_uint32), C.c_int32,
                                    C.c_int32, C.POINTER(C.c_int32), C.c_int32, C.c_int32, C.c_uint32, C.c_uint32,
                                    C.POINTER(g2s_result), C.c_char_p]),
}


def library_path():
    return os.environ.get("G2S_LIBRARY") or os.path.join(os.path.dirname(os.path.abspath(__file__)), "libg2s_hip.so")


_LIB = None


def load_library():
    global _LIB
    if _LIB is None:
        path = library_path()
        if not os.path.exists(path):
            raise OSError("%s is missing: run `python -c 'import __graft_entry__ as g; g.build()'` "
                          "(hipcc, gfx950). There is no CPU fallback." % path)
        lib = C.CDLL(path)
        for name, (res, args) in _SIGS.items():
            fn = getattr(lib, name)
            fn.restype = res
            fn.argtypes = args
        _LIB = lib
    return _LIB


def _check(rc):
    if rc != G2S_OK:
        raise G2SError(rc, (load_library().g2s_last_error() or b"").decode("utf-8", "replace"))


def _take_text(ptr):
    lib = load_library()
    if not ptr:
        return ""
    s = C.string_at(ptr).decode("ascii")
    lib.g2s_free(ptr)
    return s


class G2S:

    @staticmethod
    def device_count():
        return load_library().g2s_device_count()

    @staticmethod
    def synth_genome(length, variant, seed):
        out = _VP()
        _check(load_library().g2s_synth_genome(length, variant, seed, C.byref(out)))
        return _take_text(out)

    @staticmethod
    def synth_gaps(reads_fasta, k, fuz, ngaps, min_len, max_len, seed):
        out = _VP()
        _check(load_library().g2s_synth_gaps(reads_fasta.encode("ascii"), k, fuz, ngaps, min_len, max_len, seed,
                                             C.byref(out)))
        return _take_text(out)


def cut_scaffolds(scaffolds_text, k=31, fuz=10, mask=False, no_split=False, labels=("scaffolds.fa", "contigs.fa", "gaps.fa", "gaps.bed")):
    outs = [_VP(), _VP(), _VP(), _VP()]
    _check(load_library().g2s_cut_scaffolds(scaffolds_text.encode("ascii"), k, fuz, int(mask), int(no_split),
                                            *[x.encode() for x in labels], *[C.byref(o) for o in outs]))
    return tuple(_take_text(o) for o in outs)


def merge_scaffolds(contigs_text, gaps_text, labels=("merged.fa", "contigs.fa", "filled.fa")):
    out, log = _VP(), _VP()
    _check(load_library().g2s_merge_scaffolds(contigs_text.encode("ascii"), gaps_text.encode("ascii"),
                                              *[x.encode() for x in labels], C.byref(out), C.byref(log)))
    return _take_text(out), _take_text(log)


def filter_reads(bam, mean, std_dev, scaffold, breakpoint, gap_length=-1, flank_length=-1, unmapped_only=False,
                 threads=0):
    lib = load_library()
    o = g2s_filter_opts(mean, std_dev, breakpoint, gap_length, flank_length, int(unmapped_only), threads,
                        scaffold.encode())
    outs = [_VP(), _VP(), _VP()]
    ext, tot = C.c_int64(0), C.c_int64(0)
    tail = [C.byref(o)] + [C.byref(x) for x in outs] + [C.byref(ext), C.byref(tot)]
    if isinstance(bam, (bytes, bytearray)):
        rc = lib.g2s_filter_reads_mem(bytes(bam), len(bam), *tail)
    else:
        rc = lib.g2s_filter_reads(str(bam).encode(), *tail)
# ... 675 lines not shown
                _check(lib.g2s_team_fill(hs, len(sessions), arr, len(gaps), group_size, res, C.cast(arena.p, C.c_char_p), nbytes, C.byref(t)))
                raw = arena.raw
                out = [FillResult(res[i], raw) for i in range(len(gaps))]
            finally:
                arena.free()
                rbuf.free()
            return (out, t) if want_timing else out
        arena = C.create_string_buffer(max(1, nbytes))
        res = (g2s_result * max(1, len(gaps)))()
        prepared = (arr, keep, arena, res, nbytes)
    arr, keep, arena, res, nbytes = prepared
    hs = (_VP * len(sessions))(*[s.h for s in sessions])
    t = g2s_timing()
    _check(lib.g2s_team_fill(hs, len(sessions), arr, len(gaps), group_size, res, arena, nbytes, C.byref(t)))
    if want_timing == "raw":
        return prepared, t
    raw = arena.raw
    out = [FillResult(res[i], raw) for i in range(len(gaps))]
    return (out, t) if want_timing else out


class PreparedBatch:
    def __init__(self, session, gaps):
        lib = load_library()
        self.session = session
        self.n = len(gaps)
        self._arr, self._keep = _gap_array(gaps)
        self.h = _VP()
        _check(lib.g2s_batch_prepare(session.h, self._arr, self.n, C.byref(self.h)))
        self.nbytes = lib.g2s_batch_arena_bytes(self.h)
        self.arena = C.create_string_buffer(max(1, self.nbytes))
        self.res = (g2s_result * max(1, self.n))()

    def run(self):
        _check(load_library().g2s_batch_run(self.h, self.res, self.arena, self.nbytes))

    def timing(self):
        t = g2s_timing()
        _check(load_library().g2s_batch_timing(self.h, C.byref(t)))
        return t

    def results(self):
        raw = self.arena.raw
        return [FillResult(self.res[i], raw) for i in range(self.n)]

    def free(self):
        if self.h:
            load_library().g2s_batch_free(self.h)
            self.h = None


def test_post_gap(graph, params, gap, states, c_count, lengths, reached_j, final_d, seed, skip):
    lib = load_library()
    arr, keep = _gap_array([gap])
    n = len(states)
    nodes = (C.c_uint32 * max(1, n))(*[s[0] for s in states])
    depths = (C.c_int32 * max(1, n))(*[s[1] for s in states])
    counts = (C.c_uint32 * max(1, n))(*[s[2] for s in states])
    lens = (C.c_int32 * 2)(*(list(lengths) + [0, 0])[:2])
    res = g2s_result()
    buf = C.create_string_buffer(gap.gap_len + graph.k + params.d_err + gap.lmf + gap.rmf + 3)
    _check(lib.g2s_test_post_gap(graph.h, C.byref(params), arr, n, nodes, depths, counts, c_count, len(lengths), lens,
                                 reached_j, final_d, seed, skip, C.byref(res), buf))
    return FillResult(res, buf.raw)


def test_post_closure(graph, params, gap, records, xp, c_count, lengths, reached_j, final_d, seed, skip):
    lib = load_library()
    arr, keep = _gap_array([gap])
    n = len(records)
    flat = (C.c_uint32 * max(1, 4 * n))()
    for i, (node, cnt, meta, pred) in enumerate(records):
        flat[4 * i], flat[4 * i + 1], flat[4 * i + 2], flat[4 * i + 3] = node, cnt, meta, pred & 0xFFFFFFFF
    xs = (C.c_uint64 * max(1, len(xp)))(*xp)
    lens = (C.c_int32 * 2)(*(list(lengths) + [0, 0])[:2])
    res = g2s_result()
    buf = C.create_string_buffer(gap.gap_len + graph.k + params.d_err + gap.lmf + gap.rmf + 3)
    _check(lib.g2s_test_post_closure(graph.h, C.byref(params), arr, n, flat, len(xp), xs, c_count, len(lengths), lens,
                                     reached_j, final_d, seed, skip, C.byref(res), buf))
    return FillResult(res, buf.raw)


def test_post_segments(graph, params, gap, segs, c_count, lengths, reached_j, final_d, seed, skip):
    lib = load_library()
    arr, keep = _gap_array([gap])
    flat = (C.c_uint32 * max(1, 8 * len(segs)))()
    for i, rec in enumerate(segs):
        for q in range(8):
            flat[8 * i + q] = rec[q] & 0xFFFFFFFF
    lens = (C.c_int32 * 2)(*(list(lengths) + [0, 0])[:2])
    res = g2s_result()
    on = C.c_int32(0)
    buf = C.create_string_buffer(gap.gap_len + graph.k + params.d_err + gap.lmf + gap.rmf + 3)
    _check(lib.g2s_test_post_segments(graph.h, C.byref(params), arr, len(segs), flat, c_count, len(lengths), lens,
                                      reached_j, final_d, seed, skip, C.byref(res), buf, C.byref(on)))
    return FillResult(res, buf.raw), bool(on.value)


def test_seg_expand(graph, params, gap, segs, lengths, reached_j, n_records, n_xp):
    lib = load_library()
    arr, keep = _gap_array([gap])
    flat = (C.c_uint32 * max(1, 8 * len(segs)))()
    for i, rec in enumerate(segs):
        for q in range(8):
            flat[8 * i + q] = rec[q] & 0xFFFFFFFF
    lens = (C.c_int32 * 2)(*(list(lengths) + [0, 0])[:2])
    out = (C.c_uint32 * max(1, 4 * n_records))()
    xs = (C.c_uint64 * max(1, n_xp))()
    _check(lib.g2s_test_seg_expand(graph.h, C.byref(params), arr, len(segs), flat, len(lengths), lens, reached_j,
                                   n_records, out, n_xp, xs))
    recs = [(out[4 * i], out[4 * i + 1], out[4 * i + 2], out[4 * i + 3] - (1 << 32) if out[4 * i + 3] >> 31 else out[4 * i + 3])
            for i in range(n_records)]
    return recs, sorted(xs[i] for i in range(n_xp))


def test_graph_tables(graph):
    n = graph.num_kmers
    succ = (C.c_uint32 * max(1, 8 * n))()
    words = (C.c_uint64 * max(1, (n + 63) // 64))()
    _check(load_library().g2s_test_graph_tables(graph.h, succ, words))
    return succ, words


def test_worker_pool(threads, rounds, n):
    _check(load_library().g2s_test_worker_pool(threads, rounds, n))


def test_group_queue(nworkers, n, group_size):
    owner = (C.c_int32 * max(1, n))()
    _check(load_library().g2s_test_group_queue(nworkers, n, group_size, owner))
    return [owner[i] for i in range(n)]


def test_device_rand(device, seed, skip, n):
    out = (C.c_int32 * max(1, n))()
    _check(load_library().g2s_test_device_rand(device, seed, skip, n, out))
    return [out[i] for i in range(n)]


def test_d3_tables(device, segs, n_len, len0, len1, start_seg, rnd, base, R, dmin, dspread):
    flat = [w for s in segs for w in s]
    sa = (C.c_uint32 * max(1, len(flat)))(*flat)
    ra = (C.c_uint32 * max(1, len(rnd)))(*rnd)
    ent, bad, anom = (C.c_uint16 * (R + 1))(), (C.c_uint8 * (R + 1))(), C.c_uint32()
    _check(load_library().g2s_test_d3_tables(device, sa, len(segs), n_len, len0, len1, start_seg, ra, len(rnd), base, R, dmin,
                                             dspread, ent, bad, C.byref(anom)))
    return list(ent), list(bad), anom.value


def test_d3_chain_launches():
    return int(load_library().g2s_test_d3_chain_launches())


def test_group_queue_slow(nworkers, n, group_size, slow_worker, slow_us):
    owner = (C.c_int32 * max(1, n))()
    _check(load_library().g2s_test_group_queue_slow(nworkers, n, group_size, slow_worker, slow_us, owner))
    return [owner[i] for i in range(n)]


def test_rand_skip(seed, skip, n):
    out = (C.c_int32 * max(1, n))()
    _check(load_library().g2s_test_rand_skip(seed, skip, n, out))
    return [out[i] for i in range(n)]


def test_rand_stream(seed, skip, n):
    out = (C.c_int32 * max(1, n))()
    _check(load_library().g2s_test_rand_stream(seed, skip, n, out))
    return [out[i] for i in range(n)]


def reach_radius(gap, d_err):
    return max(0, gap.gap_len + d_err) + gap.lmf + gap.rmf


def test_last_pool_reach():
    a, b, d = C.c_uint64(), C.c_uint64(), C.c_uint64()
    known, on = C.c_int(), C.c_int()
    lv = C.c_uint32()
    _check(load_library().g2s_test_last_pool_reach(C.byref(a), C.byref(b), C.byref(known), C.byref(d), C.byref(lv), C.byref(on)))
    return dict(reach_sets=a.value, full_kmers=b.value if known.value else None, kept_kmers=d.value, levels=lv.value,
                on_device=on.value)


def test_seg_back_record(graph, device, node):
    out = (C.c_uint32 * 5)()
    _check(load_library().g2s_test_seg_back_record(graph.h, device, node, out))
    return list(out[:4]), out[4]


def test_last_pool_build():
    a, b, c, d = C.c_uint64(), C.c_uint64(), C.c_uint64(), C.c_int()
    _check(load_library().g2s_test_last_pool_build(C.byref(a), C.byref(b), C.byref(c), C.byref(d)))
    return dict(own_positions=a.value, shared_positions=b.value, keys_sorted=c.value, on_device=d.value)


def test_last_solid_count():
    pos, mx, so = C.c_uint64(), C.c_uint64(), C.c_uint64()
    ps, rf, on = C.c_uint32(), C.c_uint32(), C.c_int()
    _check(load_library().g2s_test_last_solid_count(C.byref(pos), C.byref(ps), C.byref(rf), C.byref(mx), C.byref(so), C.byref(on)))
    return dict(positions=pos.value, passes=ps.value, refined_bins=rf.value, max_pass_keys=mx.value, solid=so.value,
                on_device=on.value)


def test_plan_passes(hist, cap):
    nb = len(hist)
    h = (C.c_uint64 * max(1, nb))(*hist)
    first = (C.c_uint32 * max(1, nb))()
    n, over = C.c_uint32(), C.c_uint32()
    _check(load_library().g2s_test_plan_passes(h, nb, cap, first, nb, C.byref(n), C.byref(over)))
    assert n.value <= nb
    return list(first[:n.value]), (over.value if over.value < nb else None)


def test_filter_join(ref_id, pos, end, flag, h_own, h_mate, max_span, bits, windows, max_pairs, device=-1, threads=1):
    lib = load_library()
    nr, n = len(pos), len(windows) // 3
    assert len(windows) == 3 * n and all(len(x) == nr for x in (ref_id, end, flag, h_own, h_mate))
    flat = [v for w in windows for v in w]
    args = [(C.c_int32 * max(1, nr))(*ref_id), (C.c_int32 * max(1, nr))(*pos), (C.c_int64 * max(1, nr))(*end),
            (C.c_uint32 * max(1, nr))(*flag), (C.c_uint64 * max(1, nr))(*h_own), (C.c_uint64 * max(1, nr))(*h_mate)]
    win = (C.c_int64 * max(1, len(flat)))(*flat)
    cap1 = cap2 = 1 << 16
    while True:
        l1, l2 = (C.c_uint64 * cap1)(), (C.c_uint64 * cap2)()
        n1, n2 = C.c_uint64(0), C.c_uint64(0)
        rc = lib.g2s_test_filter_join(device, threads, nr, *args, max_span, bits, n, win, max_pairs, l1, cap1,
                                      C.byref(n1), l2, cap2, C.byref(n2))
        if rc != G2S_OK or (n1.value <= cap1 and n2.value <= cap2):
            break
        cap1, cap2 = max(cap1, n1.value), max(cap2, n2.value)
    msg = (lib.g2s_filter_last_error() or b"").decode("utf-8", "replace")
    return rc, [(x >> 32, x & 0xFFFFFFFF) for x in l1[:n1.value]], [(x >> 32, x & 0xFFFFFFFF) for x in l2[:n2.value]], msg


def reads_text(data, device=-1, piece_bytes=0):
    lib = load_library()
    data = bytes(data)
    cap = max(1 << 12, 2 * len(data))
    while True:
        out = (C.c_uint8 * cap)()
        n = C.c_size_t(0)
        _check(lib.g2s_test_reads_text(data, len(data), device, piece_bytes, out, cap, C.byref(n)))
        if n.value <= cap:
            return bytes(out[:n.value])
        cap = n.value


def last_reads_load():
    f, rb, ps, rc, pc, gr = (C.c_uint64() for _ in range(6))
    on = C.c_int()
    _check(load_library().g2s_test_last_reads_load(C.byref(f), None, None, None, None, None, None, 0, None))
    how = (C.c_int * max(1, f.value))()
    _check(load_library().g2s_test_last_reads_load(C.byref(f), C.byref(rb), C.byref(ps), C.byref(rc), C.byref(pc), C.byref(on),
                                                   how, f.value, C.byref(gr)))
    return dict(files=f.value, raw_bytes=rb.value, positions=ps.value, records=rc.value, pieces=pc.value,
                on_device=on.value, inflate=[("none", "zlib", "device", "mixed", "device-gzip")[x] for x in how[:f.value]], grows=gr.value)


BAM_READS_REASONS = ("kernels", "not asked", "rows anomaly", "over the cap", "hip")


def last_reads_bam():
    f, kept, skipped = C.c_uint64(), C.c_uint64(), C.c_uint64()
    kernels, reason, anomaly = C.c_int(), C.c_int(), C.c_int()
    _check(load_library().g2s_test_last_reads_bam(C.byref(f), C.byref(kept), C.byref(skipped), C.byref(kernels),
                                                  C.byref(reason), C.byref(anomaly)))
    return dict(files=f.value, kept=kept.value, skipped=skipped.value, kernels=kernels.value,
                reason=BAM_READS_REASONS[reason.value], anomaly=anomaly.value)


def last_reads_bam_stream():
    f, w, peak = C.c_uint64(), C.c_uint64(), C.c_uint64()
    _check(load_library().g2s_test_last_reads_bam_stream(C.byref(f), C.byref(w), C.byref(peak)))
    return dict(streamed_files=f.value, windows=w.value, peak_device_bytes=peak.value)


GZIP_OUTCOMES = ("done", "too few starts", "boundary mismatch", "slot full", "corrupt", "trailer", "memory", "hip", "header")


def set_device_gzip(mode=1):
    return load_library().g2s_reads_set_device_gzip(int(mode))


def gzip_inflate(data, device=-1, chunk_bytes=0, window_chunks=0):
    lib = load_library()
    data = bytes(data)
    cap = max(1 << 16, 8 * len(data))
    while True:
        out = (C.c_uint8 * cap)()
        n, oc = C.c_size_t(0), C.c_int(0)
        _check(lib.g2s_test_gzip_inflate(data, len(data), device, chunk_bytes, window_chunks, out, cap, C.byref(n), C.byref(oc)))
        if n.value <= cap:
            return bytes(out[:n.value]), GZIP_OUTCOMES[oc.value]
        cap = n.value


def last_reads_gzip():
    v = [C.c_uint64() for _ in range(7)]
    oc = C.c_int()
    _check(load_library().g2s_test_last_reads_gzip(C.byref(v[0]), C.byref(v[1]), C.byref(v[2]), C.byref(v[3]), C.byref(v[4]),
                                                   C.byref(v[5]), C.byref(oc), C.byref(v[6])))
    return dict(files=v[0].value, windows=v[1].value, chunks=v[2].value, starts_found=v[3].value, absorbed=v[4].value,
                members=v[5].value, outcome=GZIP_OUTCOMES[oc.value], peak_device_bytes=v[6].value)


# ... 134 lines not shown
```

Measured before the change: 3.286 million.

## Fuse D3 classify, scan and table build into one front_tables kernel

Adds a fused g2s_d3_front_tables kernel that runs gap classification, the layout scan and table construction in a single launch. It keeps per-gap records and variant descriptors in LDS instead of writing them to global memory between kernels. The kernel is used on the chained small-gap route when the LDS budget fits. This removes launches and global round trips between stages, at the cost of redundant classification per workgroup and a large dynamic LDS allocation.

```diff
diff --git a/gap2seq_amd/csrc/d3_device.h b/gap2seq_amd/csrc/d3_device.h
--- a/gap2seq_amd/csrc/d3_device.h
+++ b/gap2seq_amd/csrc/d3_device.h
@@ -164,5 +164,6 @@
                           uint16_t* entries, uint8_t* bad, uint32_t* anomalies);
 
 uint64_t d3_chain_launches();
+uint64_t d3_fused_launches();
 
 }
diff --git a/gap2seq_amd/csrc/d3_device.hip b/gap2seq_amd/csrc/d3_device.hip
--- a/gap2seq_amd/csrc/d3_device.hip
+++ b/gap2seq_amd/csrc/d3_device.hip
@@ -71,84 +71,88 @@
   return lo + (mid << 24) + (hi << 48);
 }
 
-__device__ __forceinline__ uint32_t d3_classify_body(const D3Params& P, const D3Work& W, const GapOut* __restrict__ outs,
-                                                     const D3Gap* __restrict__ dgaps, uint32_t first, uint32_t stride,
-                                                     uint32_t* l_gi, uint32_t* l_dm, uint32_t* l_ds, int32_t* l_sk,
-                                                     unsigned long long* red, bool one_wg) {
-  const uint32_t n = P.n;
+struct D3ClassAcc {
   unsigned long long xA = 0, sA = 0, xB = 0, sB = 0, xD = 0, sD = 0, segs = 0;
   uint32_t unhandled = 0, seg_gaps = 0, big = 0, traced = 0, spec = 0, handoff = 0;
-  for (uint32_t i = first; i < n; i += stride) {
-    const D3Gap dg = dgaps[i];
-    const GapOut& go = outs[i];
-    const uint32_t flags = go.flags, n_states = go.n_states, n_right = go.n_right, x_right = go.x_right, x_left = go.x_left;
-    const uint32_t x_sub = go.x_sub, n_sub = go.n_sub, nseg_b = go.stat[3], dflags = go.dflags, stop0 = go.stop[0], stop1 = go.stop[1];
-    const int c_count = go.c_count, n_len = go.n_len, len0 = go.len[0], len1 = go.len[1], reached_j = go.reached_j, count_s = go.count_s;
-    const uint32_t n_xl = go.n_xl;
-    const uint64_t sub_off = go.sub_off;
-    uint32_t gi = 0, dmin = 0, spread = 0;
-    if (dg.kind != 0) gi = GI_BAD;
+};
+struct D3GapClass {
+  uint32_t gi, dmin, spread;
+  int32_t skip_thr;
+  uint4 h0;
+  uint64_t sub_at;
+  uint32_t ns, start_seg, start_t;
+  int32_t len0, len1, n_len;
+};
+template <bool WITH_VAR>
+__device__ __forceinline__ D3GapClass d3_classify_gap(const D3Params& P, const GapOut* __restrict__ outs, const D3Gap* __restrict__ dgaps, uint32_t i,
+                                                      D3ClassAcc& A) {
+  const D3Gap dg = dgaps[i];
+  const GapOut& go = outs[i];
+  const uint32_t flags = go.flags, n_states = go.n_states, n_right = go.n_right, x_right = go.x_right, x_left = go.x_left;
+  const uint32_t x_sub = go.x_sub, n_sub = go.n_sub, nseg_b = go.stat[3], dflags = go.dflags, stop0 = go.stop[0], stop1 = go.stop[1];
+  const int c_count = go.c_count, n_len = go.n_len, len0 = go.len[0], len1 = go.len[1], reached_j = go.reached_j, count_s = go.count_s;
+  const uint32_t n_xl = go.n_xl;
+  const uint64_t sub_off = go.sub_off;
+  D3GapClass C;
+  if (WITH_VAR) { C.start_seg = go.start_seg; C.start_t = go.start_t; }
+  uint32_t gi = 0, dmin = 0, spread = 0;
+  if (dg.kind != 0) gi = GI_BAD;
+  else {
+    if (flags & (G2S_DEV_OVERFLOW_A | G2S_DEV_OVERFLOW_B)) A.unhandled++;
+    else if ((uint64_t)n_states > P.max_states || (uint64_t)n_right > P.max_states) gi = GI_MEM;
     else {
-      if (flags & (G2S_DEV_OVERFLOW_A | G2S_DEV_OVERFLOW_B)) unhandled++;
-      else if ((uint64_t)n_states > P.max_states || (uint64_t)n_right > P.max_states) gi = GI_MEM;
-      else {
-        xA += x_right; sA += n_right; xB += x_left; sB += n_states; xD += x_sub; sD += n_sub;
-        segs += nseg_b;
-        seg_gaps++;
-        if (flags & G2S_DEV_BIG) big++;
-        if (dflags & G2S_DEVA_TRACED) traced++;
-        if (dflags & G2S_DEVA_SPEC) spec++;
-        const bool phase_d = c_count > 0 && n_len > 0;
-        const bool by_host = phase_d && !(dflags & (G2S_DEVA_ANALYSED | G2S_DEVA_D2_PENDING));
-        const int cnt = (phase_d && !P.skip_confident && P.all_paths) ? count_s : c_count;
-        if (cnt > 0 && (!P.unique_paths || cnt == 1)) gi |= GI_FILLED;
-        if (n_len > 0) gi |= ((uint32_t)reached_j & 0xFFu) << 8;
-        if (phase_d) {
-          gi |= GI_PHASE_D;
-          if (by_host) gi |= GI_HOST;
-          if (by_host || (!P.skip_confident && (dflags & G2S_DEVA_D2_PENDING))) handoff++;
-          int lo_d = 0x7FFFFFFF, hi_d = 0;
-#pragma unroll
-          for (int q = 0; q < 2; q++) {
-            if (q >= n_len) continue;
-            const uint32_t sw = q ? stop1 : stop0;
-            const int lq = q ? len1 : len0;
-            int lo = (int)(sw & 0xFFFFu), hi = (int)(sw >> 16);
-            if (lo > hi || hi > (int)dg.lmf) { lo = 0; hi = (int)dg.lmf; }
-            lo_d = min(lo_d, 1 + lq - hi);
-            hi_d = max(hi_d, 1 + lq - lo);
-          }
-          lo_d = max(lo_d, 1);
-          hi_d = max(hi_d, lo_d);
-          dmin = (uint32_t)lo_d;
-          spread = (uint32_t)(hi_d - lo_d);
-          gi |= spread ? 2u : 1u;
+      A.xA += x_right; A.sA += n_right; A.xB += x_left; A.sB += n_states; A.xD += x_sub; A.sD += n_sub;
+      A.segs += nseg_b;
+      A.seg_gaps++;
+      if (flags & G2S_DEV_BIG) A.big++;
+      if (dflags & G2S_DEVA_TRACED) A.traced++;
+      if (dflags & G2S_DEVA_SPEC) A.spec++;
+      const bool phase_d = c_count > 0 && n_len > 0;
+      const bool by_host = phase_d && !(dflags & (G2S_DEVA_ANALYSED | G2S_DEVA_D2_PENDING));
+      const int cnt = (phase_d && !P.skip_confident && P.all_paths) ? count_s : c_count;
+      if (cnt > 0 && (!P.unique_paths || cnt == 1)) gi |= GI_FILLED;
+      if (n_len > 0) gi |= ((uint32_t)reached_j & 0xFFu) << 8;
+      if (phase_d) {
+        gi |= GI_PHASE_D;
+        if (by_host) gi |= GI_HOST;
+        if (by_host || (!P.skip_confident && (dflags & G2S_DEVA_D2_PENDING))) A.handoff++;
+        int lo_d = 0x7FFFFFFF, hi_d = 0;
+#pragma unroll
+        for (int q = 0; q < 2; q++) {
+          if (q >= n_len) continue;
+          const uint32_t sw = q ? stop1 : stop0;
+          const int lq = q ? len1 : len0;
+          int lo = (int)(sw & 0xFFFFu), hi = (int)(sw >> 16);
+          if (lo > hi || hi > (int)dg.lmf) { lo = 0; hi = (int)dg.lmf; }
+          lo_d = min(lo_d, 1 + lq - hi);
+          hi_d = max(hi_d, 1 + lq - lo);
         }
-      }
-    }
-    gi |= (uint32_t)dg.lmf << 16;
-    W.ginfo[i] = gi;
-    W.dmin[i] = dmin;
-    W.dspread[i] = spread;
-    W.skip[i] = dg.skip_thr;
-    if (l_gi) { l_gi[i] = gi; l_dm[i] = dmin; l_ds[i] = spread; l_sk[i] = dg.skip_thr; }
-    uint4 h0;
-    const uint64_t ao = P.arena_base + dg.arena_off, sa = (uint64_t)(i / P.group_size) * P.sub_region + sub_off;
-    h0.x = (uint32_t)ao; h0.y = (uint32_t)(ao >> 32); h0.z = (uint32_t)sa; h0.w = (uint32_t)(sa >> 32);
-    ((uint4*)&W.tdesc[i])[0] = h0;
-    (void)n_xl;
-  }
-  xA = wave_add64(xA); sA = wave_add64(sA); xB = wave_add64(xB); sB = wave_add64(sB); xD = wave_add64(xD); sD = wave_add64(sD);
-  segs = wave_add64(segs);
-  const unsigned long long cnts = wave_add64(((unsigned long long)unhandled << 32) | seg_gaps);
-  big = dpp_sum(big);
-  if ((threadIdx.x & 63u) == 0u && big) atomicAdd(&W.sum->big_gaps, big);
-  traced = dpp_sum(traced);
-  if ((threadIdx.x & 63u) == 0u && traced) atomicAdd(&W.sum->traced_gaps, traced);
-  spec = dpp_sum(spec);
-  if ((threadIdx.x & 63u) == 0u && spec) atomicAdd(&W.sum->spec_gaps, spec);
-  handoff = dpp_sum(handoff);
-  if ((threadIdx.x & 63u) == 0u && handoff) atomicAdd(&W.sum->handoff_gaps, handoff);
+        lo_d = max(lo_d, 1);
+        hi_d = max(hi_d, lo_d);
+        dmin = (uint32_t)lo_d;
+        spread = (uint32_t)(hi_d - lo_d);
+        gi |= spread ? 2u : 1u;
+      }
+    }
+  }
+  gi |= (uint32_t)dg.lmf << 16;
+  C.gi = gi; C.dmin = dmin; C.spread = spread; C.skip_thr = dg.skip_thr;
+  const uint64_t ao = P.arena_base + dg.arena_off, sa = (uint64_t)(i / P.group_size) * P.sub_region + sub_off;
+  C.h0.x = (uint32_t)ao; C.h0.y = (uint32_t)(ao >> 32); C.h0.z = (uint32_t)sa; C.h0.w = (uint32_t)(sa >> 32);
+  C.sub_at = sa; C.ns = n_xl; C.len0 = len0; C.len1 = len1; C.n_len = n_len;
+  return C;
+}
+__device__ __forceinline__ uint32_t d3_classify_sums(const D3Work& W, const D3ClassAcc& A, unsigned long long* red, bool one_wg, bool store) {
+  const unsigned long long xA = wave_add64(A.xA), sA = wave_add64(A.sA), xB = wave_add64(A.xB), sB = wave_add64(A.sB), xD = wave_add64(A.xD), sD = wave_add64(A.sD);
+  const unsigned long long segs = wave_add64(A.segs);
+  const unsigned long long cnts = wave_add64(((unsigned long long)A.unhandled << 32) | A.seg_gaps);
+  const uint32_t big = dpp_sum(A.big), traced = dpp_sum(A.traced), spec = dpp_sum(A.spec), handoff = dpp_sum(A.handoff);
+  if (store && (threadIdx.x & 63u) == 0u) {
+    if (big) atomicAdd(&W.sum->big_gaps, big);
+    if (traced) atomicAdd(&W.sum->traced_gaps, traced);
+    if (spec) atomicAdd(&W.sum->spec_gaps, spec);
+    if (handoff) atomicAdd(&W.sum->handoff_gaps, handoff);
+  }
   const uint32_t wave = threadIdx.x >> 6, nwaves = blockDim.x >> 6;
   if ((threadIdx.x & 63u) == 0u) {
     unsigned long long* r = red + wave * 8u;
@@ -160,6 +164,7 @@
   unsigned long long all_cnts = 0;
   for (uint32_t w = 0; w < nwaves; w++) all_cnts += red[w * 8u + 7u];
   D3Summary* S = W.sum;
+  if (!store) return (uint32_t)(all_cnts >> 32);
   if (threadIdx.x < 7u) {
     unsigned long long* dst = (unsigned long long*)&S->xA + threadIdx.x;
     if (one_wg) *dst = tot; else if (tot) atomicAdd(dst, tot);
@@ -171,6 +176,23 @@
     }
   }
   return (uint32_t)(all_cnts >> 32);
+}
+__device__ __forceinline__ uint32_t d3_classify_body(const D3Params& P, const D3Work& W, const GapOut* __restrict__ outs,
+                                                     const D3Gap* __restrict__ dgaps, uint32_t first, uint32_t stride,
+                                                     uint32_t* l_gi, uint32_t* l_dm, uint32_t* l_ds, int32_t* l_sk,
+                                                     unsigned long long* red, bool one_wg) {
+  const uint32_t n = P.n;
+  D3ClassAcc A;
+  for (uint32_t i = first; i < n; i += stride) {
+    const D3GapClass C = d3_classify_gap<false>(P, outs, dgaps, i, A);
+    W.ginfo[i] = C.gi;
+    W.dmin[i] = C.dmin;
+    W.dspread[i] = C.spread;
+    W.skip[i] = C.skip_thr;
+    if (l_gi) { l_gi[i] = C.gi; l_dm[i] = C.dmin; l_ds[i] = C.spread; l_sk[i] = C.skip_thr; }
+    ((uint4*)&W.tdesc[i])[0] = C.h0;
+  }
+  return d3_classify_sums(W, A, red, one_wg, true);
 }
 __global__ __launch_bounds__(256) void g2s_d3_classify(const D3Params P, const D3Work W, const GapOut* __restrict__ outs,
                                                        const D3Gap* __restrict__ dgaps) {
@@ -206,7 +228,8 @@
   const uint32_t ia = dpp_scan_add(a), ib = dpp_scan_add(b), ic = dpp_scan_sat(c);
   if (lane == 63) { sh[wave * 3] = ia; sh[wave * 3 + 1] = ib; sh[wave * 3 + 2] = ic; }
   __syncthreads();
-  uint32_t wa = lane < 16 ? sh[lane * 3] : 0u, wb = lane < 16 ? sh[lane * 3 + 1] : 0u, wc = lane < 16 ? sh[lane * 3 + 2] : 0u;
+  const int nwaves = (int)(blockDim.x >> 6);
+  uint32_t wa = lane < nwaves ? sh[lane * 3] : 0u, wb = lane < nwaves ? sh[lane * 3 + 1] : 0u, wc = lane < nwaves ? sh[lane * 3 + 2] : 0u;
   wa = dpp_scan_add(wa); wb = dpp_scan_add(wb); wc = dpp_scan_sat(wc);
   *tot_a = (uint32_t)__builtin_amdgcn_readlane((int)wa, 15); *tot_b = (uint32_t)__builtin_amdgcn_readlane((int)wb, 15);
   *tot_c = (uint32_t)__builtin_amdgcn_readlane((int)wc, 15);
@@ -218,11 +241,15 @@
   c = incl_c == 0xFFFFFFFFu ? 0xFFFFFFFFu : incl_c - c;
 }
 
-__device__ __forceinline__ void d3_scan_body(const D3Params& P, const D3Work& W, const GapOut* __restrict__ outs, uint32_t* gi_a,
+struct D3Layout { uint32_t status, V, tiles; uint64_t T; };
+template <uint32_t NT = 1024u>
+__device__ __forceinline__ D3Layout d3_scan_body(const D3Params& P, const D3Work& W, const GapOut* __restrict__ outs, uint32_t* gi_a,
                                              uint32_t* dm_a, uint32_t* ds_a, const int32_t* sk_a, bool dual, uint32_t unhandled,
-                                             uint64_t* sh , uint32_t* sh_f , bool short_list ) {
+                                             uint64_t* sh , uint32_t* sh_f , bool short_list ,
+                                             bool store = true, uint4* l_vd = nullptr) {
+  static_assert(NT == 1024u || NT == 256u, "the skip rule's composition: NT / 64 ranges a lane");
   const uint32_t t = threadIdx.x, n = P.n;
-  const uint32_t per = (n + 1023u) / 1024u;
+  const uint32_t per = (n + NT - 1u) / NT;
   const uint32_t lo = min(n, t * per), hi = min(n, lo + per);
   if (P.has_skip) {
     auto s_of = [&](uint32_t i) -> bool {
@@ -237,9 +264,10 @@
     sh_f[t] = (o0 ? 1u : 0u) | (o1 ? 2u : 0u);
     __syncthreads();
     if (t < 64u) {
+      constexpr uint32_t FQ = NT / 64u;
       auto apply = [](uint32_t f, bool in) -> bool { return in ? (f & 2u) != 0 : (f & 1u) != 0; };
       uint32_t f = 2u;
-      for (uint32_t q = 0; q < 16u; q++) { const uint32_t g = sh_f[t * 16u + q]; f = (apply(g, apply(f, false)) ? 1u : 0u) | (apply(g, apply(f, true)) ? 2u : 0u); }
+      for (uint32_t q = 0; q < FQ; q++) { const uint32_t g = sh_f[t * FQ + q]; f = (apply(g, apply(f, false)) ? 1u : 0u) | (apply(g, apply(f, true)) ? 2u : 0u); }
       uint32_t inc = f;
       for (int o = 1; o < 64; o <<= 1) {
         const uint32_t pv = (uint32_t)__shfl_up((int)inc, o);
@@ -248,7 +276,7 @@
       uint32_t before = (uint32_t)__shfl_up((int)inc, 1);
       if (t == 0) before = 2u;
       bool cur = apply(before, false);
-      for (uint32_t q = 0; q < 16u; q++) { const uint32_t g = sh_f[t * 16u + q]; sh_f[t * 16u + q] = cur ? 1u : 0u; cur = apply(g, cur); }
+      for (uint32_t q = 0; q < FQ; q++) { const uint32_t g = sh_f[t * FQ + q]; sh_f[t * FQ + q] = cur ? 1u : 0u; cur = apply(g, cur); }
     }
     __syncthreads();
     bool sk = sh_f[t] != 0;
@@ -257,7 +285,7 @@
       if (sk) {
         const uint32_t g = (gi_a[i] & ~3u) | GI_SKIPPED;
         gi_a[i] = g; dm_a[i] = 0; ds_a[i] = 0;
-        if (dual) { W.ginfo[i] = g; W.dmin[i] = 0; W.dspread[i] = 0; }
+        if (dual && store) { W.ginfo[i] = g; W.dmin[i] = 0; W.dspread[i] = 0; }
       }
     }
     __threadfence_block();
@@ -273,7 +301,7 @@
       s8[q] = have ? ds_a[i] : 0u;
     }
   };
-  if (t == 0) stamp(W, 20);
+  if (t == 0 && store) stamp(W, 20);
   uint64_t sd = 0, ss = 0;
   uint32_t nv = 0;
   for (uint32_t i0 = lo; i0 < hi; i0 += 8u) {
@@ -293,7 +321,7 @@
     block_scan3_short(a, b, nv, (uint32_t*)sh, &ta, &tb, &V);
     sd = a; ss = b; tot_d = ta; tot_s = tb;
   } else block_scan3(sd, ss, nv, sh, &tot_d, &tot_s, &V);
-  if (t == 0) stamp(W, 21);
+  if (t == 0 && store) stamp(W, 21);
   const bool too_wide = tot_d + tot_s + P.base0 + P.R0 >= 0xFFFF0000ull || tot_s + P.R0 >= (uint64_t)G2S_D3_TABLE_BUDGET;
   uint64_t my_tab = 0, my_blk = 0;
   uint32_t my_tiles = 0;
@@ -307,13 +335,11 @@
       for (int q = 0; q < 8; q++) {
         const uint32_t i = i0 + (uint32_t)q;
         if (i >= hi) break;
-        W.base[i] = (uint32_t)d;
-        W.vrank[i] = v;
+        if (store) { W.base[i] = (uint32_t)d; W.vrank[i] = v; }
         if (g8[q] & GI_SKIPPED) continue;
         d += m8[q];
         if (GI_CLASS(g8[q]) == 2u) {
-          W.var_gap[v] = i;
-          W.var_R[v] = (uint32_t)r;
+          if (store) { W.var_gap[v] = i; W.var_R[v] = (uint32_t)r; }
           my_tab += r + 1u;
           my_tiles += (uint32_t)((r + D3_TILE) / D3_TILE);
           if (v % G2S_D3_BLOCK_VARS == 0u) my_blk += r + 1u;
@@ -322,9 +348,9 @@
         }
       }
     }
-    if (t == 1023u) W.var_R[V] = (uint32_t)tot_s + P.R0;
-  }
-  if (t == 0) stamp(W, 22);
+    if (t == NT - 1u && store) W.var_R[V] = (uint32_t)tot_s + P.R0;
+  }
+  if (t == 0 && store) stamp(W, 22);
   uint64_t to = my_tab, bo = my_blk, T, TB;
   uint32_t tl = my_tiles, tiles;
   if (short_list) {
@@ -345,27 +371,26 @@
         const uint32_t base_i = (uint32_t)d;
         d += m8[q];
         if (GI_CLASS(g8[q]) != 2u) continue;
-        W.var_toff[v] = (uint32_t)to;
-        W.var_tile[v] = tl;
+        if (store) { W.var_toff[v] = (uint32_t)to; W.var_tile[v] = tl; }
         {
           const uint32_t i = i0 + (uint32_t)q;
           uint4 h0, h1;
           h0.x = i; h0.y = (uint32_t)r; h0.z = (uint32_t)to; h0.w = tl;
           h1.x = base_i; h1.y = m8[q]; h1.z = s8[q]; h1.w = 0u;
-          ((uint4*)&W.vdesc[v])[0] = h0;
-          ((uint4*)&W.vdesc[v])[1] = h1;
+          if (l_vd) { l_vd[2u * v] = h0; l_vd[2u * v + 1u] = h1; }
+          else { ((uint4*)&W.vdesc[v])[0] = h0; ((uint4*)&W.vdesc[v])[1] = h1; }
         }
         tl += (uint32_t)((r + D3_TILE) / D3_TILE);
         to += r + 1u;
-        if (v % G2S_D3_BLOCK_VARS == 0u) { W.blk_toff[v / G2S_D3_BLOCK_VARS] = (uint32_t)bo; bo += r + 1u; }
+        if (v % G2S_D3_BLOCK_VARS == 0u) { if (store) W.blk_toff[v / G2S_D3_BLOCK_VARS] = (uint32_t)bo; bo += r + 1u; }
         v++;
         r += s8[q];
       }
     }
-    if (t == 1023u) { W.var_toff[V] = (uint32_t)T; W.var_tile[V] = tiles; W.blk_toff[(V + G2S_D3_BLOCK_VARS - 1u) / G2S_D3_BLOCK_VARS] = (uint32_t)TB; }
+    if (t == NT - 1u && store) { W.var_toff[V] = (uint32_t)T; W.var_tile[V] = tiles; W.blk_toff[(V + G2S_D3_BLOCK_VARS - 1u) / G2S_D3_BLOCK_VARS] = (uint32_t)TB; }
     __threadfence_block();
     __syncthreads();
-    for (uint32_t v = t; v < V; v += 1024u) {
+    for (uint32_t v = t; v < V && !l_vd; v += NT) {
       const uint4 h0 = ((const uint4*)&W.vdesc[v])[0];
       const uint32_t i = h0.x, r = h0.y, tl0 = h0.w;
       const GapOut& go = outs[i];
@@ -380,7 +405,10 @@
       for (uint32_t x = 0; x < nt; x++) W.tile_var[tl0 + x] = v;
     }
   }
-  if (t == 0) {
+  D3Layout L;
+  L.status = (unhandled ? G2S_D3_UNHANDLED : 0u) | (over ? G2S_D3_BUDGET : 0u);
+  L.V = V; L.tiles = over ? 0u : tiles; L.T = T;
+  if (t == 0 && store) {
     stamp(W, 23);
     D3Summary* S = W.sum;
     S->status = (unhandled ? G2S_D3_UNHANDLED : 0u) | (over ? G2S_D3_BUDGET : 0u);
@@ -391,6 +419,7 @@
     S->draws_min = tot_d;
     S->draws_spread = tot_s;
   }
+  return L;
 }
 #define D3_SCAN_LDS_GAPS 12288u
 __global__ __launch_bounds__(1024) void g2s_d3_scan(const D3Params P, const D3Work W, const GapOut* __restrict__ outs) {
@@ -402,10 +431,10 @@
     for (uint32_t i = threadIdx.x; i < P.n; i += 1024u) { l_gi[i] = W.ginfo[i]; l_dm[i] = W.dmin[i]; l_ds[i] = W.dspread[i]; }
     const uint32_t unhandled = W.sum->unhandled;
     __syncthreads();
-    d3_scan_body(P, W, outs, l_gi, l_dm, l_ds, W.skip, true, unhandled, sh, sh_f, true);
+    (void)d3_scan_body(P, W, outs, l_gi, l_dm, l_ds, W.skip, true, unhandled, sh, sh_f, true);
     return;
   }
-  d3_scan_body(P, W, outs, W.ginfo, W.dmin, W.dspread, W.skip, false, W.sum->unhandled, sh, sh_f, P.n <= 262144u);
+  (void)d3_scan_body(P, W, outs, W.ginfo, W.dmin, W.dspread, W.skip, false, W.sum->unhandled, sh, sh_f, P.n <= 262144u);
 }
 
 __global__ __launch_bounds__(64) void g2s_rand_window(uint32_t* __restrict__ Wd, const uint32_t* __restrict__ link) {
@@ -904,8 +933,161 @@
   const uint32_t unhandled = d3_classify_body(P, W, outs, dgaps, threadIdx.x, 1024u, l_gi, l_dm, l_ds, l_sk, red, true);
   __syncthreads();
   if (threadIdx.x == 0) stamp(W, 1);
-  d3_scan_body(P, W, outs, l_gi, l_dm, l_ds, l_sk, true, unhandled, sh, sh_f, true);
+  (void)d3_scan_body(P, W, outs, l_gi, l_dm, l_ds, l_sk, true, unhandled, sh, sh_f, true);
   if (threadIdx.x == 0) stamp(W, 2);
+}
+
+#define D3_FUSED_GRID 256u
+#define D3_FUSED_GAPS 768u
+#define D3_FUSED_GAP_BYTES 80u
+__global__ __launch_bounds__(256) void g2s_d3_front_tables(const D3Params P, const D3Work W, const GapOut* __restrict__ outs,
+                                                           const D3Gap* __restrict__ dgaps, const SubRec* __restrict__ sub,
+                                                           const uint32_t* __restrict__ rnd , uint64_t capacity) {
+  __shared__ __attribute__((aligned(16))) uint32_t lraw[D3_TAB_SEGS * 4u];
+  __shared__ uint64_t sh[96];
+  __shared__ unsigned long long red[4 * 8];
+  __shared__ uint32_t sh_f[256];
+  extern __shared__ __attribute__((aligned(16))) uint32_t dyn[];
+  SegLite* lseg = (SegLite*)lraw;
+  const uint32_t n = P.n, tid = threadIdx.x;
+  uint4* l_go = (uint4*)dyn;
+  uint4* l_vd = l_go + 2u * n;
+  uint32_t *l_gi = (uint32_t*)(l_vd + 2u * n), *l_dm = l_gi + n, *l_ds = l_dm + n;
+  int32_t* l_sk = (int32_t*)(l_ds + n);
+  uint32_t* lwin = (uint32_t*)(l_sk + n);
+  const bool wg0 = blockIdx.x == 0, st0 = wg0 && tid == 0;
+  if (st0) stamp(W, 0);
+  D3ClassAcc A;
+  {
+    constexpr uint32_t Q = (D3_FUSED_GAPS + 255u) / 256u;
+    D3GapClass C[Q];
+    D3ClassAcc a[Q];
+#pragma unroll
+    for (uint32_t q = 0; q < Q; q++) C[q] = d3_classify_gap<true>(P, outs, dgaps, min(tid + 256u * q, n - 1u), a[q]);
+#pragma unroll
+    for (uint32_t q = 0; q < Q; q++) {
+      const uint32_t i = tid + 256u * q;
+      if (i >= n) continue;
+      A.xA += a[q].xA; A.sA += a[q].sA; A.xB += a[q].xB; A.sB += a[q].sB; A.xD += a[q].xD; A.sD += a[q].sD; A.segs += a[q].segs;
+      A.unhandled += a[q].unhandled; A.seg_gaps += a[q].seg_gaps; A.big += a[q].big; A.traced += a[q].traced; A.spec += a[q].spec;
+      A.handoff += a[q].handoff;
+      l_gi[i] = C[q].gi; l_dm[i] = C[q].dmin; l_ds[i] = C[q].spread; l_sk[i] = C[q].skip_thr;
+      uint4 g0, g1;
+      g0.x = (uint32_t)C[q].sub_at; g0.y = (uint32_t)(C[q].sub_at >> 32); g0.z = C[q].start_seg; g0.w = C[q].start_t;
+      g1.x = (uint32_t)C[q].len0; g1.y = (uint32_t)C[q].len1; g1.z = (uint32_t)C[q].n_len; g1.w = C[q].ns;
+      l_go[2u * i] = g0; l_go[2u * i + 1u] = g1;
+      if (wg0) {
+        W.ginfo[i] = C[q].gi; W.dmin[i] = C[q].dmin; W.dspread[i] = C[q].spread; W.skip[i] = C[q].skip_thr;
+        ((uint4*)&W.tdesc[i])[0] = C[q].h0;
+      }
+    }
+  }
+  const uint32_t unhandled = d3_classify_sums(W, A, red, true, wg0);
+  __syncthreads();
+  if (st0) stamp(W, 1);
+  const D3Layout L = d3_scan_body<256u>(P, W, outs, l_gi, l_dm, l_ds, l_sk, true, unhandled, sh, sh_f, true, wg0, l_vd);
+  __syncthreads();
+  if (st0) { stamp(W, 2); stamp(W, 3); }
+  if (L.status) return;
+  if (st0) stamp(W, 4);
+  const uint32_t win_cap = P.map_cap + D3_TILE;
+  const uint32_t V = L.V, tiles = L.tiles, T = (uint32_t)L.T;
+  const uint32_t lane = tid & 63u;
+  auto find_v = [&](uint32_t x, int word) -> uint32_t {
+    uint32_t cnt = 0;
+    for (uint32_t v0 = 0; v0 < V; v0 += 64u) {
+      const uint32_t v = v0 + lane;
+      const uint4 h = l_vd[2u * min(v, V - 1u)];
+      cnt += (uint32_t)__popcll(__ballot(v < V && (word == 2 ? h.z : h.w) <= x));
+    }
+    return uni(max(cnt, 1u) - 1u);
+  };
+  const bool by_wave = tiles <= D3_WAVE_TILES;
+  bool bad_any = false, worked = false;
+  if (by_wave) {
+    const uint32_t wave = uni(tid >> 6);
+    uint16_t *jmp = (uint16_t*)lraw + wave * 2u * D3_TAB_SEGS, *dep = jmp + D3_TAB_SEGS;
+    const bool stw = blockIdx.x == gridDim.x - 1u && tid == 0;
+    for (uint32_t e = (gridDim.x - 1u - blockIdx.x) * 4u + wave; e < T; e += gridDim.x * 4u) {
+      const uint32_t v = find_v(e, 2);
+      const uint4 h0 = l_vd[2u * v], h1 = l_vd[2u * v + 1u];
+      const uint32_t i = uni(h0.x);
+      const uint4 g0 = l_go[2u * i], g1 = l_go[2u * i + 1u];
+      const uint32_t toff = uni(h0.z), base = uni(h1.x), dmin = h1.y, dspread = h1.z, ns = uni(g1.w);
+      const uint32_t d = e - toff;
+      if (stw) stamp(W, 5);
+      if (ns > D3_TAB_SEGS) continue;
+      worked = true;
+      const uint64_t sub_at = (uint64_t)uni(g0.x) | ((uint64_t)uni(g0.y) << 32);
+      const uint64_t at = (uint64_t)base + d;
+      bool bad = false;
+      const int draws = d3_count_wave((int)uni(g1.z), (int)g1.x, (int)g1.y, g0.z, ns, (const SegW*)(sub + sub_at), rnd + at,
+                                      min(win_cap, dmin + dspread + 1u), capacity > at ? capacity - at : 0ull, jmp, dep, &bad);
+      if (stw) stamp(W, 6);
+      const int dev = draws - (int)dmin;
+      if (dev < 0 || dev > (int)dspread) bad = true;
+      if (lane == 0u) {
+        W.tab[(uint64_t)e] = bad ? (uint16_t)0 : (uint16_t)dev;
+        if (W.tab_bad) W.tab_bad[(uint64_t)e] = bad ? 1 : 0;
+        bad_any |= bad;
+      }
+    }
+  }
+  for (uint32_t tile = blockIdx.x; tile < tiles; tile += gridDim.x) {
+    const uint32_t v = find_v(tile, 3);
+    const uint4 h0 = l_vd[2u * v], h1 = l_vd[2u * v + 1u];
+    const uint32_t i = uni(h0.x);
+    const uint4 g0 = l_go[2u * i], g1 = l_go[2u * i + 1u];
+    g2s::D3Var vd;
+    vd.gap = i; vd.R = uni(h0.y); vd.toff = uni(h0.z); vd.tile0 = uni(h0.w); vd.base = uni(h1.x); vd.dmin = uni(h1.y); vd.dspread = uni(h1.z); vd.ns = uni(g1.w);
+    vd.sub_at = (uint64_t)uni(g0.x) | ((uint64_t)uni(g0.y) << 32); vd.start_seg = uni(g0.z); vd.start_t = uni(g0.w);
+    vd.len0 = (int32_t)uni(g1.x); vd.len1 = (int32_t)uni(g1.y); vd.n_len = (int32_t)uni(g1.z);
+    const uint32_t ns = vd.ns;
+    if (by_wave && ns <= D3_TAB_SEGS) continue;
+    worked = true;
+    const uint32_t d0 = (tile - vd.tile0) * D3_TILE, d = d0 + tid;
+    const uint64_t at0 = (uint64_t)vd.base + d0;
+    const bool mine = d <= vd.R;
+    const uint32_t want = min(win_cap, min(vd.R - d0, D3_TILE - 1u) + vd.dmin + vd.dspread + 1u);
+    if (st0 && !by_wave) stamp(W, 5);
+    __syncthreads();
+    {
+      const SegW* gs = (const SegW*)(sub + vd.sub_at);
+      const uint32_t in_lds = ns <= D3_TAB_SEGS ? ns : 0u;
+#pragma unroll
+      for (uint32_t it = 0; it < D3_TAB_SEGS / 256u; it++) {
+        const uint32_t q = tid + 256u * it;
+        if (q >= in_lds) continue;
+        SegLite l;
+        l.depth_len = gs[q].depth_len; l.par01 = gs[q].par01; l.par23 = gs[q].par23; l.flags = gs[q].flags;
+        lseg[q] = l;
+      }
+      for (uint32_t x = tid; x < want; x += 256u) lwin[x] = at0 + x < capacity ? rnd[at0 + x] : 0u;
+    }
+    __syncthreads();
+    if (st0 && !by_wave) stamp(W, 6);
+    if (mine) {
+      bool bad = false;
+      const uint64_t at = at0 + tid;
+      const uint32_t nw = want > tid ? want - tid : 0u;
+      const uint64_t av = capacity > at ? capacity - at : 0ull;
+      const int draws = ns > D3_TAB_SEGS
+                            ? d3_walk_count(vd.n_len, vd.len0, vd.len1, vd.start_seg, vd.start_t, (int)ns, (const SegW*)(sub + vd.sub_at), lwin + tid, nw, av, &bad)
+                            : d3_walk_count_lite(vd.n_len, vd.len0, vd.len1, vd.start_seg, (int)ns, lseg, lwin + tid, nw, av, &bad);
+      const int dev = draws - (int)vd.dmin;
+      if (dev < 0 || dev > (int)vd.dspread) bad = true;
+      W.tab[(uint64_t)vd.toff + d] = bad ? (uint16_t)0 : (uint16_t)dev;
+      if (W.tab_bad) W.tab_bad[(uint64_t)vd.toff + d] = bad ? 1 : 0;
+      bad_any |= bad;
+    }
+  }
+  if (bad_any) atomicAdd(&W.sum->anomalies, 1u);
+  if (st0) stamp(W, 7);
+  if (P.laps && lane == 0u) {
+    unsigned long long* laps = (unsigned long long*)((char*)W.sum + 512);
+    if (worked) atomicMax(&laps[32], wall_clock64());
+    if (tid == 0) atomicMax(&laps[33], wall_clock64());
+  }
 }
 
 template <bool RESTART>
@@ -1925,6 +2107,24 @@
 
 static std::atomic<uint64_t> chain_launches{0};
 uint64_t d3_chain_launches() { return chain_launches.load(std::memory_order_relaxed); }
+static std::atomic<uint64_t> fused_launches{0};
+uint64_t d3_fused_launches() { return fused_launches.load(std::memory_order_relaxed); }
+
+static bool launch_front_tables(hipStream_t st, const D3Params& P, const D3Work& W, const GapOut* outs, const D3Gap* dgaps, const SubRec* sub,
+                                uint32_t* rnd_all, uint64_t rnd_capacity) {
+  const size_t lds = (size_t)P.n * D3_FUSED_GAP_BYTES + ((size_t)P.map_cap + D3_TILE) * 4;
+  if (lds > 144u * 1024u) return false;
+  if (hipFuncSetAttribute((const void*)g2s_d3_front_tables, hipFuncAttributeMaxDynamicSharedMemorySize, (int)lds) != hipSuccess) {
+    (void)hipGetLastError();
+    return false;
+  }
+  uint32_t grid = D3_FUSED_GRID;
+  const char* grid_s = GENV("G2S_TEST_FUSED_GRID");
+  if (grid_s) grid = std::min(grid, (uint32_t)std::max(atoi(grid_s), 1));
+  hipLaunchKernelGGL(g2s_d3_front_tables, dim3(grid), dim3(256), lds, st, P, W, outs, dgaps, sub, rnd_all + 31, rnd_capacity);
+  fused_launches.fetch_add(1, std::memory_order_relaxed);
+  return true;
+}
 
 hipError_t launch_d3(hipStream_t st, const D3Params& P, const D3Work& W, const GapDev* gaps, const GapOut* outs,
                      const D3Gap* dgaps, const SubRec* sub, const char* lastch_up, const char* lastch_dn,
@@ -1938,7 +2138,20 @@
   hipError_t e = summary_is_clean ? hipSuccess : hipMemsetAsync(W.sum, 0, 1024 + 64 * 128, st);
   if (e != hipSuccess) return e;
   const bool short_list = P.n <= D3_FRONT_GAPS;
-  if (P.restart) {
+  const char* waves_s = GENV("G2S_TRACE_WAVES");
+  const int waves_env = waves_s ? atoi(waves_s) : 0;
+  const bool four = waves_env ? waves_env == 4 : P.n <= 768u;
+  const bool chain_route = !P.restart && four && P.n <= D3_CHAIN_GAPS && ev_chain == nullptr && P.group_size >= P.n && !P.base0 && !P.R0 && !P.d_in;
+  static_assert(D3_CHAIN_GAPS <= D3_FUSED_GAPS, "g2s_d3_front_tables classifies D3_FUSED_GAPS / 256 gaps a thread");
+  const char* back_s = chain_route ? GENV("G2S_D3_BACK") : nullptr;
+  const bool chain_in_trace = chain_route && !(back_s && atoi(back_s) != 0);
+  bool fused = false;
+  if (chain_in_trace) {
+    const char* front_s = GENV("G2S_D3_FRONT");
+    if (!(front_s && atoi(front_s) != 0)) fused = launch_front_tables(st, P, W, outs, dgaps, sub, rnd_all, rnd_capacity);
+  }
+  if (fused) {
+  } else if (P.restart) {
     if (ev_d2) { e = hipStreamWaitEvent(st, ev_d2, 0); if (e != hipSuccess) return e; }
     hipLaunchKernelGGL(g2s_d3_restart, dim3((P.n + 255u) / 256u), dim3(256), 0, st, P, W, outs, dgaps, sub, rnd_all + 31, rnd_capacity, side);
   } else if (short_list) hipLaunchKernelGGL(g2s_d3_front, dim3(1), dim3(1024), 0, st, P, W, outs, dgaps);
@@ -1946,18 +2159,12 @@
     hipLaunchKernelGGL(g2s_d3_classify, dim3((P.n + 255u) / 256u), dim3(256), 0, st, P, W, outs, dgaps);
     launch_scan(st, P, W, outs);
   }
-  if (!P.restart) { e = launch_tables(st, P, W, sub, rnd_all, rnd_capacity); if (e != hipSuccess) return e; }
+  if (!P.restart && !fused) { e = launch_tables(st, P, W, sub, rnd_all, rnd_capacity); if (e != hipSuccess) return e; }
   if (ev_d2 && short_list && !P.restart) { e = hipStreamWaitEvent(st, ev_d2, 0); if (e != hipSuccess) return e; }
-  const char* waves_s = GENV("G2S_TRACE_WAVES");
-  const int waves_env = waves_s ? atoi(waves_s) : 0;
-  const bool four = waves_env ? waves_env == 4 : P.n <= 768u;
   const size_t lds = (size_t)P.seg_cap * (sizeof(SegRec) + 16) + (size_t)P.map_cap * 8 + 16;
-  bool chain_in_trace = false;
   uint32_t chain_room = 0;
   static_assert(D3_CHAIN_GAPS <= 768u, "g2s_d3_trace<4, true> is the four-wave kernel");
-  if (!P.restart && four && P.n <= D3_CHAIN_GAPS && ev_chain == nullptr && P.group_size >= P.n && !P.base0 && !P.R0 && !P.d_in) {
-    const char* back_s = GENV("G2S_D3_BACK");
-    chain_in_trace = !(back_s && atoi(back_s) != 0);
+  if (chain_route) {
     const char* room_s = GENV("G2S_TEST_CHAIN_ROOM");
     chain_room = (uint32_t)std::min<size_t>(lds / 2u, 0x7FFFFFFFu);
     if (room_s) chain_room = std::min(chain_room, (uint32_t)std::max(atoi(room_s), 0));
diff --git a/gap2seq_amd/csrc/g2s_api.hip b/gap2seq_amd/csrc/g2s_api.hip
--- a/gap2seq_amd/csrc/g2s_api.hip
+++ b/gap2seq_amd/csrc/g2s_api.hip
@@ -5048,6 +5048,7 @@
 }
 
 extern "C" uint64_t g2s_test_d3_chain_launches(void) { return d3_chain_launches(); }
+extern "C" uint64_t g2s_test_d3_fused_launches(void) { return d3_fused_launches(); }
 
 extern "C" int g2s_test_rand_skip(uint32_t seed, uint64_t skip, uint32_t n, int32_t* out) {
   if (!out) return fail(G2S_ERR_ARG, "g2s_test_rand_skip: bad argument");
diff --git a/gap2seq_amd/lib.py b/gap2seq_amd/lib.py
--- a/gap2seq_amd/lib.py
+++ b/gap2seq_amd/lib.py
@@ -237,6 +237,7 @@
                                      C.POINTER(C.c_uint32), C.c_uint64, C.c_uint32, C.c_uint32, C.c_uint32, C.c_uint32,
                                      C.POINTER(C.c_uint16), C.POINTER(C.c_uint8), C.POINTER(C.c_uint32)]),
     "g2s_test_d3_chain_launches": (C.c_uint64, []),
+    "g2s_test_d3_fused_launches": (C.c_uint64, []),
     "g2s_test_post_closure": (C.c_int, [_VP, C.POINTER(g2s_params), C.POINTER(g2s_gap), C.c_uint32,
                                         C.POINTER(C.c_uint32), C.c_uint32, C.POINTER(C.c_uint64), C.c_int32, C.c_int32,
                                         C.POINTER(C.c_int32), C.c_int32, C.c_int32, C.c_uint32, C.c_uint64,
@@ -1218,6 +1219,10 @@
     return int(load_library().g2s_test_d3_chain_launches())
 
 
+def test_d3_fused_launches():
+    return int(load_library().g2s_test_d3_fused_launches())
+
+
 def test_group_queue_slow(nworkers, n, group_size, slow_worker, slow_us):
     owner = (C.c_int32 * max(1, n))()
     _check(load_library().g2s_test_group_queue_slow(nworkers, n, group_size, slow_worker, slow_us, owner))
```

Result: no change. 3.255 million (-0.9%).
